# facebookresearch/SlowFast

Measured on NVIDIA H100. Metric: clips/sec (fwd+bwd) SlowFast-8x8-R50, higher is better.
Workload: dtype bf16x3-split operands, f32 accumulate/storage

## Files before the change

include/slowfast_b200.h:

```cpp
#ifndef SLOWFAST_B200_H_
#define SLOWFAST_B200_H_

#include <stdint.h>

#ifdef __cplusplus
extern "C" {
#endif

const char* sfb_last_error(void);
int sfb_abi_version(void);
const char* sfb_build_arch(void);

typedef struct sfb_conv_desc {
  const void* a_hi;
  const void* a_lo;
  int32_t n, d, h, w, c;
  int64_t c_pitch;
  const void* b_hi;
  const void* b_lo;
  int32_t cout;
  int32_t kt, kh, kw;
  int32_t dil_t, dil_h, dil_w;
  int32_t str_t, str_h, str_w;
  int32_t low_t, low_h, low_w;
  int32_t out_t, out_h, out_w;
  float* out;
  int64_t os_n, os_t, os_h, os_w;
  int32_t accumulate;
  float* stats;
  int32_t nsplit;
} sfb_conv_desc;

int64_t sfb_conv_m_tiles(const sfb_conv_desc* d);
int32_t sfb_conv_ksplit(const sfb_conv_desc* d);
int sfb_conv_igemm(const sfb_conv_desc* d, void* stream);

typedef struct sfb_wgrad_desc {
  const void* x_hi;
  const void* x_lo;
  int32_t n, d, h, w, c;
  int64_t c_pitch;
  const void* dy_hi;
  const void* dy_lo;
  int32_t cout;
  int64_t dy_pitch;
  int32_t kt, kh, kw;
  int32_t dil_t, dil_h, dil_w;
  int32_t str_t, str_h, str_w;
  int32_t low_t, low_h, low_w;
  int32_t out_t, out_h, out_w;
  float* dw;
  int32_t nsplit;
} sfb_wgrad_desc;

int sfb_conv_wgrad(const sfb_wgrad_desc* d, void* stream);

typedef struct sfb_wgrad_plan {
  int32_t direct;
  int32_t transposed;
  int32_t tile_rows;
  int32_t bn;
  int32_t ck;
  int32_t tiles;
  int32_t k_blocks;
  int32_t slices;
  int32_t ctas;
} sfb_wgrad_plan;
int sfb_conv_wgrad_plan(const sfb_wgrad_desc* d, int32_t num_sms, sfb_wgrad_plan* out);

int sfb_set_wgrad_direct(int32_t enabled);

int sfb_zero_f32_2d(float* ptr, int64_t rows, int64_t c, int64_t pitch, void* stream);

int sfb_add_f32_2d(float* dst, const float* src, int64_t rows, int32_t c, int64_t dst_pitch, int64_t src_pitch,
                   void* stream);

int sfb_split_planes(const float* x, int64_t rows, int32_t c, int64_t x_pitch, void* hi, void* lo,
                     int64_t o_pitch, void* stream);
int sfb_input_pack(const float* x, int32_t n, int32_t c, int32_t t, int32_t h, int32_t w, int32_t c_pad, void* hi,
                   void* lo, void* stream);
int sfb_filter_pack(const float* w, int32_t cout, int32_t cin, int32_t taps_total, const int32_t* tapmap,
                    int32_t ntaps, int32_t transpose, int32_t cols_pad, void* hi, void* lo, void* stream);
int sfb_filter_unpack_grad(const float* dwm, float* dw, int32_t cout, int32_t cin, int32_t taps, int32_t cin_pad,
                           int32_t accumulate, void* stream);

int sfb_bn_finalize(const float* partials, int32_t m_tiles, int32_t c, int64_t count, const float* gamma,
                    const float* beta, float* running_mean, float* running_var, float momentum, float eps,
                    int32_t training, float* scale, float* shift, float* save_mean, float* save_invstd,
                    int32_t affine_c, void* stream);

int32_t sfb_bn_split_stats_tiles(int64_t rows, int64_t rows_per_clip, int32_t splits, int32_t c);
int sfb_bn_split_stats(const float* y, int64_t y_pitch, int64_t rows, int32_t c, int32_t splits, int64_t rows_per_clip,
                       float* partials, void* stream);

typedef struct sfb_bn_apply_desc {
  const float* y; int64_t y_pitch; const float* scale; const float* shift;
  const float* y2; int64_t y2_pitch; const float* scale2; const float* shift2;
  const void* res_hi; const void* res_lo; int64_t res_pitch;
  void* out_hi; void* out_lo; int64_t out_pitch;
  int64_t rows; int32_t c; int32_t relu;
  int32_t splits; int64_t rows_per_clip;
} sfb_bn_apply_desc;
int sfb_bn_apply(const sfb_bn_apply_desc* d, void* stream);

typedef struct sfb_bn_bwd_desc {
  const float* dout; int64_t dout_pitch;
  const void* mask_hi; int64_t mask_pitch;
  const float* y; int64_t y_pitch;
  const float* mean; const float* invstd; const float* gamma;
  float* dgamma; float* dbeta; int32_t accumulate_param_grads;
  int32_t training;
  void* dy_hi; void* dy_lo; int64_t dy_pitch;
  float* dres; int64_t dres_pitch; int32_t dres_accumulate;
  float* partials;
  float* coef;
  int64_t rows; int32_t c;
  int32_t c_valid;
  const float* mask_scale; const float* mask_shift;
  int32_t splits; int64_t rows_per_clip;
} sfb_bn_bwd_desc;
int32_t sfb_bn_bwd_blocks(int64_t rows, int32_t c, int32_t splits, int64_t rows_per_clip);
int sfb_bn_bwd(const sfb_bn_bwd_desc* d, void* stream);

typedef struct sfb_pool_desc {
  const float* y; const float* scale; const float* shift;
  int32_t n, t, h, w, c, oh, ow, kh, kw, sh, sw, ph, pw;
  void* out_hi; void* out_lo; int64_t out_pitch;
  uint8_t* argmax;
  const float* dout; int64_t dout_pitch;
  float* dz;
  int32_t splits;
} sfb_pool_desc;
int sfb_bn_relu_maxpool_fwd(const sfb_pool_desc* d, void* stream);
int sfb_bn_relu_maxpool_bwd(const sfb_pool_desc* d, void* stream);



typedef struct sfb_pool3d_desc {
  const void* in_hi; const void* in_lo; int64_t in_pitch;
  void* out_hi; void* out_lo; int64_t out_pitch;
  uint8_t* argmax;
  int32_t n, t, h, w, c, ot, oh, ow;
  int32_t kt, kh, kw, st, sh, sw, pt, ph, pw;
  const float* dout; int64_t dout_pitch;
  float* din; int64_t din_pitch; int32_t din_accumulate;
} sfb_pool3d_desc;
int sfb_maxpool3d_fwd(const sfb_pool3d_desc* d, void* stream);
int sfb_maxpool3d_bwd(const sfb_pool3d_desc* d, void* stream);

int sfb_stem_input_fold(const float* x, int32_t n, int32_t cin, int32_t t, int32_t h, int32_t w, void* hi, void* lo,
                        void* stream);
int sfb_stem_filter_fold(const float* w, float* dw, int32_t cout, int32_t cin, int32_t kt, int32_t kh, int32_t kw,
                         int32_t pad_w, int32_t kwf, void* hi, void* lo, const float* gmat, int32_t reverse,
                         void* stream);
typedef struct sfb_stem_desc {
  const void* x_hi; const void* x_lo;
  int32_t n, t, h, wf;
  const void* f_hi; const void* f_lo;
  const void* dy_hi; const void* dy_lo;
  int32_t cout, kt, kh, kwf;
  int32_t str_t, str_h, pad_t, pad_h, pad_wf;
  int32_t out_t, out_h, out_w;
  float* out;
  float* stats;
  float* dwm;
  int32_t nsplit;
} sfb_stem_desc;
int64_t sfb_stem_m_tiles(const sfb_stem_desc* d);
int sfb_stem_fprop(const sfb_stem_desc* d, void* stream);
int sfb_stem_wgrad(const sfb_stem_desc* d, void* stream);
int sfb_stem8_supported(const sfb_stem_desc* d);
int64_t sfb_stem8_m_tiles(const sfb_stem_desc* d);
int sfb_stem8_input_fold(const float* x, int32_t n, int32_t cin, int32_t t, int32_t h, int32_t w, void* hi, void* lo,
                         void* stream);
int sfb_stem8_filter_fold(const float* w, int32_t cin, int32_t kt, void* hi, void* lo, void* stream);
int sfb_stem8_fprop(const sfb_stem_desc* d, void* stream);
int sfb_stem8_wgrad(const sfb_stem_desc* d, void* stream);

typedef struct sfb_bgemm_desc {
  const void* a_hi; const void* a_lo; int64_t lda, batch_stride_a; int32_t a_mn_major;
  const void* b_hi; const void* b_lo; int64_t ldb, batch_stride_b; int32_t b_mn_major;
  int32_t m, n, k, batch;
  float* out; int64_t ldd, batch_stride_d;
  float alpha;
  int32_t accumulate;
  int32_t nsplit;
} sfb_bgemm_desc;
int sfb_gemm_batched(const sfb_bgemm_desc* d, void* stream);

int sfb_layernorm_fwd(const float* x, int64_t x_pitch, int64_t rows, int32_t c, const float* gamma, const float* beta,
                      float eps, void* o_hi, void* o_lo, float* o_f32, int64_t o_pitch, float* mean, float* rstd,
                      void* stream);
int32_t sfb_rowslab_blocks(int64_t rows);
int sfb_layernorm_bwd(const float* dy, int64_t dy_pitch, const float* x, int64_t x_pitch, int64_t rows, int32_t c,
                      const float* gamma, const float* mean, const float* rstd, float* dx, int64_t dx_pitch,
                      int32_t dx_accumulate, float* dgamma, float* dbeta, int32_t param_accumulate, float* partials,
                      void* stream);
int sfb_colsum(const float* src, int64_t pitch, int64_t rows, int32_t c, float* out, int32_t accumulate, float* partials,
               void* stream);
int sfb_tokens_assemble(const float* y, const float* bias, const float* cls, const float* pos_spatial,
                        const float* pos_temporal, const float* pos_class, int32_t b, int32_t l, int32_t hw, int32_t c,
                        float* x, void* stream);
// ... 211 lines not shown
```

slowfast_b200/csrc/conv_direct.cu:

```cuda
#include <cstdint>
#include <cuda_bf16.h>

#include "../../include/slowfast_b200.h"
#include "tmap.h"

namespace sfb {

struct DirectParams {
  const __nv_bfloat16* a_hi; const __nv_bfloat16* a_lo; int64_t c_pitch;
  const __nv_bfloat16* b_hi; const __nv_bfloat16* b_lo;
  int nb, id, ih, iw, c, cout;
  int kd, kh, kw, dd, dh, dw, sd, sh, sw, ld, lh, lw, oz, op, oq;
  int M, m_tiles, ktot, coutp;
  float* out; long long os_n, os_z, os_p, os_q; int accumulate; int ncols_store;
  float* stats;
};

__device__ __forceinline__ void dc_load8(const __nv_bfloat16* hi, const __nv_bfloat16* lo, int64_t off, float (&x)[8]) {
  const uint4 h = *reinterpret_cast<const uint4*>(hi + off);
  const uint32_t hw[4] = {h.x, h.y, h.z, h.w};
#pragma unroll
  for (int i = 0; i < 4; ++i) {
    x[2 * i] = __uint_as_float(hw[i] << 16);
    x[2 * i + 1] = __uint_as_float(hw[i] & 0xffff0000u);
// ... 49 lines not shown
          const int iw = w0 + tw * p.dw;
          if (id < 0 || id >= p.id || ih < 0 || ih >= p.ih || iw < 0 || iw >= p.iw) continue;
          const int64_t base = (((int64_t(on_) * p.id + id) * p.ih + ih) * p.iw + iw) * p.c_pitch;
          const float* wt = wsm + size_t(tap) * p.c * COUT_T;
          for (int c0 = 0; c0 < p.c; c0 += 8) {
            float x[8];
            dc_load8(p.a_hi, p.a_lo, base + c0, x);
#pragma unroll
            for (int ci = 0; ci < 8; ++ci) {
              const float xv = x[ci];
              const float4* w4 = reinterpret_cast<const float4*>(wt + size_t(c0 + ci) * COUT_T);
#pragma unroll
              for (int j = 0; j < COUT_T / 4; ++j) {
                const float4 w = w4[j];
                acc[4 * j + 0] = fmaf(xv, w.x, acc[4 * j + 0]);
                acc[4 * j + 1] = fmaf(xv, w.y, acc[4 * j + 1]);
                acc[4 * j + 2] = fmaf(xv, w.z, acc[4 * j + 2]);
                acc[4 * j + 3] = fmaf(xv, w.w, acc[4 * j + 3]);
              }
            }
          }
        }
      }
    }
  }
  float* tile = red + 8 * COUT_T;
  long long* roff_s = reinterpret_cast<long long*>(tile + 128 * (COUT_T + 1));
#pragma unroll
  for (int j = 0; j < COUT_T; ++j) tile[threadIdx.x * (COUT_T + 1) + j] = acc[j];
  roff_s[threadIdx.x] = rvalid ? roff : -1;
  __syncthreads();
  {
    const int ncols = p.ncols_store;
    for (int e = threadIdx.x; e < 128 * ncols; e += 128) {
      int px, col;
      if (ncols == COUT_T) {
        px = e / COUT_T;
        col = e - px * COUT_T;
      } else {
        px = e / ncols;
        col = e - px * ncols;
      }
      const long long off = roff_s[px];
      if (off < 0) continue;
      float v = tile[px * (COUT_T + 1) + col];
      float* dst = p.out + off + col;
      if (p.accumulate == 2) {
        atomicAdd(dst, v);
      } else {
        if (p.accumulate) v += *dst;
        *dst = v;
      }
    }
  }
  if (p.stats == nullptr) return;
  const int lane = threadIdx.x & 31, warp = threadIdx.x >> 5;
#pragma unroll
  for (int j = 0; j < COUT_T; ++j) {
    float s = rvalid ? acc[j] : 0.f;
    float s2 = s * s;
#pragma unroll
    for (int o = 16; o > 0; o >>= 1) {
      s += __shfl_xor_sync(0xffffffffu, s, o);
      s2 += __shfl_xor_sync(0xffffffffu, s2, o);
    }
    if (lane == 0) {
      red[(warp * 2 + 0) * COUT_T + j] = s;
      red[(warp * 2 + 1) * COUT_T + j] = s2;
    }
  }
  __syncthreads();
  for (int j = threadIdx.x; j < p.cout; j += blockDim.x) {
    float s = 0.f, s2 = 0.f;
#pragma unroll
    for (int w = 0; w < 4; ++w) {
      s += red[(w * 2 + 0) * COUT_T + j];
      s2 += red[(w * 2 + 1) * COUT_T + j];
    }
    p.stats[size_t(j) * p.m_tiles + mt] = s;
    p.stats[(size_t(p.cout) + j) * p.m_tiles + mt] = s2;
  }
}

int conv_direct_try(const sfb_conv_desc* d, cudaStream_t stream, int* rc_out) {
  const int taps = d->kt * d->kh * d->kw;
  const int64_t macs = int64_t(taps) * d->c * d->cout;
  int coutp = 8;
  while (coutp < d->cout) coutp <<= 1;
  const size_t smem = (size_t(taps) * d->c * coutp + size_t(8) * coutp + size_t(128) * (coutp + 1)) * sizeof(float) +
                      128 * sizeof(long long) + 8;
  if (d->c > 8 || d->cout > 64 || macs > 1024 || smem > 96 * 1024) return 0;
  DirectParams p;
  p.a_hi = (const __nv_bfloat16*)d->a_hi; p.a_lo = (const __nv_bfloat16*)d->a_lo; p.c_pitch = d->c_pitch;
  p.b_hi = (const __nv_bfloat16*)d->b_hi; p.b_lo = (const __nv_bfloat16*)d->b_lo;
  p.nb = d->n; p.id = d->d; p.ih = d->h; p.iw = d->w; p.c = d->c; p.cout = d->cout;
  p.kd = d->kt; p.kh = d->kh; p.kw = d->kw; p.dd = d->dil_t; p.dh = d->dil_h; p.dw = d->dil_w;
  p.sd = d->str_t; p.sh = d->str_h; p.sw = d->str_w; p.ld = d->low_t; p.lh = d->low_h; p.lw = d->low_w;
  p.oz = d->out_t; p.op = d->out_h; p.oq = d->out_w;
  p.M = int(int64_t(d->n) * d->out_t * d->out_h * d->out_w);
  p.m_tiles = (p.M + 127) / 128;
  p.ktot = taps * d->c;
  p.coutp = coutp;
  p.out = d->out; p.os_n = d->os_n; p.os_z = d->os_t; p.os_p = d->os_h; p.os_q = d->os_w;
  p.accumulate = d->accumulate;
  p.ncols_store = (d->cout + 3) & ~3;
  p.stats = d->stats;
  static bool attr = false;
  if (!attr) {
    cudaFuncSetAttribute(conv_direct_kernel<8>, cudaFuncAttributeMaxDynamicSharedMemorySize, 100 * 1024);
    cudaFuncSetAttribute(conv_direct_kernel<16>, cudaFuncAttributeMaxDynamicSharedMemorySize, 100 * 1024);
    cudaFuncSetAttribute(conv_direct_kernel<32>, cudaFuncAttributeMaxDynamicSharedMemorySize, 100 * 1024);
    cudaFuncSetAttribute(conv_direct_kernel<64>, cudaFuncAttributeMaxDynamicSharedMemorySize, 100 * 1024);
    attr = true;
  }
  switch (coutp) {
    case 8: conv_direct_kernel<8><<<p.m_tiles, 128, smem, stream>>>(p); break;
    case 16: conv_direct_kernel<16><<<p.m_tiles, 128, smem, stream>>>(p); break;
    case 32: conv_direct_kernel<32><<<p.m_tiles, 128, smem, stream>>>(p); break;
    default: conv_direct_kernel<64><<<p.m_tiles, 128, smem, stream>>>(p); break;
  }
  const cudaError_t e = cudaGetLastError();
  if (e != cudaSuccess) {
    set_error("sfb_conv_igemm (direct SIMT body) launch failed: %s", cudaGetErrorString(e));
    *rc_out = -20;
  } else {
    *rc_out = 0;
  }
  return 1;
}

}
```

slowfast_b200/csrc/conv_igemm.cu:

```cuda
#include <algorithm>
#include <cstdint>
#include <cstdio>

#include "../../include/slowfast_b200.h"
#include "ptx.cuh"
#include "tmap.h"

namespace sfb {

constexpr int BLOCK_M = 128;
constexpr int MAX_STAGES = 8;
constexpr int EPI_WARPS = 8;
constexpr int EPI_STAGE_FLOATS = 64;
constexpr int MMA_WARPS = 8;
constexpr int PRODUCER_WARP = MMA_WARPS;
constexpr int EPI_WARP0 = MMA_WARPS + 1;
constexpr int CONV_THREADS = 32 * (MMA_WARPS + 1 + EPI_WARPS);
constexpr int BN_MAX = 128;
constexpr int BLOCK_K = 64;
constexpr int KSTEPS = BLOCK_K / 16;

struct ConvParams {
  CUtensorMap tmA[2];
  CUtensorMap tmB[2];
  int M, oq, op, oz, nb;
  int sw, sh, sd;
  int lw, lh, ld;
  int kw, kh, kd;
  int dw, dh, dd;
  int CK, cpt, n_chunks, cps, k_blocks;
  int Ntot, BN, n_tiles, m_tiles;
  int ksplit;
  int stages;
  int a_tiled;
  uint32_t stage_bytes, chunk_bytes, b_bytes, a_total_bytes, a_plane_bytes;
  uint32_t a_layout, a_sbo, a_lbo;
  uint32_t a_kstep[KSTEPS];
  uint32_t acc_pitch;
  uint32_t off_acc, off_staging, off_red, off_bars;
  float* out;
  long long os_n, os_z, os_p, os_q;
  int accumulate;
  int epi_coalesced;
  float* stats;
};

__device__ __forceinline__ int k_block_begin(const ConvParams& p, int kpart) {
  return kpart * p.k_blocks / p.ksplit;
}

int conv_direct_try(const sfb_conv_desc* d, cudaStream_t stream, int* rc_out);

template <int NSPLIT, int BN>
__global__ void __launch_bounds__(CONV_THREADS, 1) conv_igemm_kernel(const __grid_constant__ ConvParams p) {
  static_assert(BN % 16 == 0 && BN <= BN_MAX, "tile width: a multiple of 16 up to BN_MAX");
  extern __shared__ uint8_t smem_raw[];
  uint8_t* smem = reinterpret_cast<uint8_t*>((reinterpret_cast<uintptr_t>(smem_raw) + 1023) & ~uintptr_t(1023));

  const int warp = threadIdx.x >> 5;
  const int lane = threadIdx.x & 31;

  uint64_t* full = reinterpret_cast<uint64_t*>(smem + p.off_bars);
  uint64_t* empty = full + MAX_STAGES;
  uint64_t* tfull = empty + MAX_STAGES;
  uint64_t* tempty = tfull + 1;
  float* acc_tile = reinterpret_cast<float*>(smem + p.off_acc);

  if (threadIdx.x == 0) {
    for (int s = 0; s < p.stages; ++s) {
      mbar_init(&full[s], 1);
      mbar_init(&empty[s], 32 * MMA_WARPS);
    }
    mbar_init(tfull, 32 * MMA_WARPS);
    mbar_init(tempty, EPI_WARPS);
    fence_mbar_init();
    fence_proxy_async_smem();
  }
  __syncthreads();

  const int total_units = p.m_tiles * p.n_tiles * p.ksplit;

  if (warp == PRODUCER_WARP) {
    if (lane == 0) {
      tma_prefetch_desc(&p.tmA[0]);
      tma_prefetch_desc(&p.tmB[0]);
      if (NSPLIT == 3) {
        tma_prefetch_desc(&p.tmA[1]);
        tma_prefetch_desc(&p.tmB[1]);
      }
    }
    int stage = 0;
    uint32_t phase = 0;
    for (int unit = blockIdx.x; unit < total_units; unit += gridDim.x) {
      const int tile = unit / p.ksplit, kpart = unit - tile * p.ksplit;
      const int mt = tile / p.n_tiles, nt = tile - mt * p.n_tiles;
      const int kb0 = k_block_begin(p, kpart), kb1 = k_block_begin(p, kpart + 1);
      int t = mt * BLOCK_M;
      const int q0 = t % p.oq;
      t /= p.oq;
      const int p0 = t % p.op;
      t /= p.op;
      const int z0 = t % p.oz;
      const int n0 = t / p.oz;
      const int cw = p.lw + q0 * p.sw, ch = p.lh + p0 * p.sh, cd = p.ld + z0 * p.sd;
      for (int kb = kb0; kb < kb1; ++kb) {
        mbar_wait(&empty[stage], phase ^ 1);
        if (elect_one()) {
          const int chunk0 = kb * p.cps;
          const uint32_t bytes = (uint32_t(p.cps) * p.chunk_bytes + p.b_bytes) * (NSPLIT == 3 ? 2u : 1u);
          mbar_expect_tx(&full[stage], bytes);
          uint8_t* st = smem + size_t(stage) * p.stage_bytes;
          for (int j = 0; j < p.cps; ++j) {
            const int idx = chunk0 + j;
            int nn = p.nb, c0 = 0;
            uint16_t ow = 0, oh = 0, od = 0;
            if (idx < p.n_chunks) {
              const int tap = idx / p.cpt;
              c0 = (idx - tap * p.cpt) * p.CK;
              const int tw = tap % p.kw;
              const int t2 = tap / p.kw;
              const int th = t2 % p.kh;
              const int td = t2 / p.kh;
              ow = uint16_t(tw * p.dw);
              oh = uint16_t(th * p.dh);
              od = uint16_t(td * p.dd);
              nn = n0;
            }
            if (p.a_tiled) {
              const int row0 = idx < p.n_chunks ? mt * BLOCK_M : p.m_tiles * BLOCK_M;
              tma_load_2d(st + j * p.chunk_bytes, &p.tmA[0], &full[stage], c0, row0);
              if (NSPLIT == 3) tma_load_2d(st + p.a_plane_bytes + j * p.chunk_bytes, &p.tmA[1], &full[stage], c0, row0);
              continue;
            }
            tma_load_im2col_5d(st + j * p.chunk_bytes, &p.tmA[0], &full[stage], c0, cw, ch, cd, nn, ow, oh, od);
            if (NSPLIT == 3)
              tma_load_im2col_5d(st + p.a_plane_bytes + j * p.chunk_bytes, &p.tmA[1], &full[stage], c0, cw, ch, cd,
                                 nn, ow, oh, od);
          }
          tma_load_2d(st + p.a_total_bytes, &p.tmB[0], &full[stage], kb * 64, nt * BN);
          if (NSPLIT == 3)
            tma_load_2d(st + p.a_total_bytes + p.b_bytes, &p.tmB[1], &full[stage], kb * 64, nt * BN);
        }
        __syncwarp();
        if (++stage == p.stages) {
          stage = 0;
          phase ^= 1;
        }
      }
    }
  } else if (warp < MMA_WARPS) {
    const int g = warp >> 2;
    const uint32_t a_row_off = uint32_t(g) * 8u * p.a_sbo;
    float d[BN / 2];
    int stage = 0;
    uint32_t phase = 0;
    int it = 0;
    for (int unit = blockIdx.x; unit < total_units; unit += gridDim.x, ++it) {
      const int kpart = unit % p.ksplit;
      const int kb0 = k_block_begin(p, kpart), kb1 = k_block_begin(p, kpart + 1);
#pragma unroll
      for (int i = 0; i < BN / 2; ++i) d[i] = 0.f;
      int held = -1;
      for (int kb = kb0; kb < kb1; ++kb) {
        mbar_wait(&full[stage], phase);
        wgmma_fence();
        const uint32_t a_base = smem_u32(smem + size_t(stage) * p.stage_bytes) + a_row_off;
        const uint32_t b_base = smem_u32(smem + size_t(stage) * p.stage_bytes) + p.a_total_bytes;
        const uint64_t a_hi0 = make_smem_desc(a_base, p.a_lbo, p.a_sbo, p.a_layout);
        const uint64_t b_hi0 = make_smem_desc(b_base, 16, 1024, 2);
#pragma unroll
        for (int ks = 0; ks < KSTEPS; ++ks) {
          const uint64_t a_hi = a_hi0 + p.a_kstep[ks];
          const uint64_t b_hi = b_hi0 + uint64_t(ks * 2);
          if (NSPLIT == 3) {
            const uint64_t a_lo = a_hi + (p.a_plane_bytes >> 4);
            const uint64_t b_lo = b_hi + (p.b_bytes >> 4);
            wgmma_m64n<BN>(d, a_lo, b_hi);
            wgmma_m64n<BN>(d, a_hi, b_lo);
          }
          wgmma_m64n<BN>(d, a_hi, b_hi);
        }
        wgmma_commit();
        wgmma_wait<1>();
        if (held >= 0) mbar_arrive(&empty[held]);
        held = stage;
        if (++stage == p.stages) {
          stage = 0;
          phase ^= 1;
        }
      }
      wgmma_wait<0>();
      mbar_arrive(&empty[held]);
      mbar_wait(tempty, (it & 1) ^ 1);
      acc_store<BN>(d, BN, acc_tile + size_t(g) * 64 * p.acc_pitch, int(p.acc_pitch));
      mbar_arrive(tfull);
    }
  } else {
    const int ew = warp - EPI_WARP0;
    const int q = ew & 3;
    const int half = ew >> 2;
    long long* roff_s = reinterpret_cast<long long*>(reinterpret_cast<float*>(smem + p.off_staging) + ew * EPI_STAGE_FLOATS);
    float* red = reinterpret_cast<float*>(smem + p.off_red);
    const int sub = lane >> 2, cq = lane & 3;
    constexpr int nchunks = BN >> 4;
    const float* qtile = acc_tile + size_t(q) * 32 * p.acc_pitch;
    int it = 0;
    for (int unit = blockIdx.x; unit < total_units; unit += gridDim.x, ++it) {
      const int tile = unit / p.ksplit;
      const int acc = it & 1;
      const int mt = tile / p.n_tiles, nt = tile - mt * p.n_tiles;
      const int ncol0 = nt * BN;
      const int row = mt * BLOCK_M + q * 32 + lane;
      const bool rvalid = row < p.M;
      long long roff = 0;
      if (rvalid) {
        int t = row;
        const int oq_ = t % p.oq;
        t /= p.oq;
        const int op_ = t % p.op;
        t /= p.op;
        const int oz_ = t % p.oz;
        const int on_ = t / p.oz;
        roff = on_ * p.os_n + oz_ * p.os_z + op_ * p.os_p + oq_ * p.os_q;
      }
      const uint32_t rmask = __ballot_sync(0xffffffffu, rvalid);
      float* red_w = red + ((size_t(acc) * 4 + q) * BN) * 2;
      roff_s[lane] = roff;
      __syncwarp();
      long long ro[4];
#pragma unroll
      for (int k = 0; k < 4; ++k) ro[k] = roff_s[k * 8 + sub];

      mbar_wait(tfull, it & 1);
      for (int ch = half; ch < nchunks; ch += 2) {
        const int c0 = ch * 16;
        const int limit = min(BN, p.Ntot - ncol0) - c0;
        const bool cvalid = cq * 4 < limit;
        float s4[4] = {0.f, 0.f, 0.f, 0.f}, q4[4] = {0.f, 0.f, 0.f, 0.f};
#pragma unroll
        for (int k = 0; k < 4; ++k) {
          const int r = k * 8 + sub;
          const float4 y = *reinterpret_cast<const float4*>(qtile + size_t(r) * p.acc_pitch + c0 + cq * 4);
          s4[0] += y.x; s4[1] += y.y; s4[2] += y.z; s4[3] += y.w;
          q4[0] = fmaf(y.x, y.x, q4[0]); q4[1] = fmaf(y.y, y.y, q4[1]);
          q4[2] = fmaf(y.z, y.z, q4[2]); q4[3] = fmaf(y.w, y.w, q4[3]);
          if (((rmask >> r) & 1u) && cvalid) {
            float4* dst = reinterpret_cast<float4*>(p.out + ro[k] + ncol0 + c0 + cq * 4);
            if (p.accumulate == 2) {
              asm volatile("red.global.add.v4.f32 [%0], {%1, %2, %3, %4};" ::"l"(dst), "f"(y.x), "f"(y.y), "f"(y.z), "f"(y.w)
                           : "memory");
            } else if (p.accumulate) {
              const float4 o = *dst;
              *dst = make_float4(y.x + o.x, y.y + o.y, y.z + o.z, y.w + o.w);
            } else {
              *dst = y;
            }
          }
        }
        if (p.stats != nullptr) {
#pragma unroll
          for (int i = 0; i < 4; ++i) {
#pragma unroll
            for (int o = 4; o <= 16; o <<= 1) {
              s4[i] += __shfl_xor_sync(0xffffffffu, s4[i], o);
              q4[i] += __shfl_xor_sync(0xffffffffu, q4[i], o);
            }
          }
          if (sub == 0) {
#pragma unroll
            for (int i = 0; i < 4; ++i) {
              const int cl = c0 + cq * 4 + i;
              red_w[cl * 2 + 0] = s4[i];
              red_w[cl * 2 + 1] = q4[i];
            }
          }
        }
      }
      __syncwarp();
      if (lane == 0) mbar_arrive(tempty);
      if (p.stats != nullptr) {
        named_bar_sync(1, 32 * EPI_WARPS);
        const float* rb = red + size_t(acc) * 4 * BN * 2;
        for (int cl = ew * 32 + lane; cl < BN; cl += 32 * EPI_WARPS) {
          const int col = ncol0 + cl;
          if (col < p.Ntot) {
            float s = 0.f, s2 = 0.f;
#pragma unroll
            for (int w = 0; w < 4; ++w) {
              s += rb[(size_t(w) * BN + cl) * 2 + 0];
              s2 += rb[(size_t(w) * BN + cl) * 2 + 1];
            }
            p.stats[size_t(col) * p.m_tiles + mt] = s;
            p.stats[(size_t(p.Ntot) + col) * p.m_tiles + mt] = s2;
          }
        }
      }
    }
  }

}

static int g_num_sms = 0;
static int g_smem_optin = 0;

static int device_props() {
  if (g_num_sms) return 0;
  int dev = 0;
  if (cudaGetDevice(&dev) != cudaSuccess) {
    set_error("cudaGetDevice failed: no CUDA device");
    return -1;
  }
  cudaDeviceGetAttribute(&g_num_sms, cudaDevAttrMultiProcessorCount, dev);
  cudaDeviceGetAttribute(&g_smem_optin, cudaDevAttrMaxSharedMemoryPerBlockOptin, dev);
  return 0;
}

static int pick_ck(int c) {
  if (c % 64 == 0) return 64;
  if (c % 32 == 0) return 32;
  if (c % 16 == 0) return 16;
  return 8;
}

struct ConvGrid {
  int64_t M;
  int CK, cps, n_chunks, k_blocks, BN, m_tiles, n_tiles;
};
static ConvGrid conv_grid(const sfb_conv_desc* d) {
  ConvGrid g;
  g.M = int64_t(d->n) * d->out_t * d->out_h * d->out_w;
  g.CK = pick_ck(d->c);
  g.cps = BLOCK_K / g.CK;
  g.n_chunks = d->kt * d->kh * d->kw * (d->c / g.CK);
  g.k_blocks = (g.n_chunks + g.cps - 1) / g.cps;
  g.BN = std::min((d->cout + 15) / 16 * 16, BN_MAX);
  g.m_tiles = int((g.M + BLOCK_M - 1) / BLOCK_M);
  g.n_tiles = (d->cout + g.BN - 1) / g.BN;
  return g;
}

static bool rows_regular(const sfb_conv_desc* d) {
  return d->os_h == int64_t(d->out_w) * d->os_w && d->os_t == int64_t(d->out_h) * d->os_h &&
         d->os_n == int64_t(d->out_t) * d->os_t;
}

static int conv_ksplit(const sfb_conv_desc* d, const ConvGrid& g, bool with_stats) {
  const int tiles = g.m_tiles * g.n_tiles;
  const int P = g_num_sms;
  if (P <= 0 || d->c <= 8 || 2 * tiles < P) return 1;
  if ((d->accumulate == 0 || with_stats) && !rows_regular(d)) return 1;
  if (with_stats && (d->accumulate != 0 || d->cout % 8 != 0 || d->os_w % 4 != 0)) return 1;
  auto cost = [&](int s) { return double((int64_t(tiles) * s + P - 1) / P) / s * (1.0 + 0.02 * (s - 1)); };
  int best = 1;
  for (int s = 2; s <= 8 && 4 * s <= g.k_blocks; ++s)
    if (cost(s) < cost(best)) best = s;
  return cost(best) < 0.9 * cost(1) ? best : 1;
}

}

using namespace sfb;

extern "C" int64_t sfb_conv_m_tiles(const sfb_conv_desc* d) {
  const ConvGrid g = conv_grid(d);
  if (device_props() == 0 && conv_ksplit(d, g, true) > 1)
    return sfb_bn_split_stats_tiles(g.M, g.M, 1, d->cout);
  return g.m_tiles;
}

extern "C" int32_t sfb_conv_ksplit(const sfb_conv_desc* d) {
  if (device_props()) return 1;
  return conv_ksplit(d, conv_grid(d), d->stats != nullptr);
}

extern "C" int sfb_conv_igemm(const sfb_conv_desc* d, void* stream_) {
  cudaStream_t stream = reinterpret_cast<cudaStream_t>(stream_);
  if (device_props()) return -1;
  if (d->nsplit != 1 && d->nsplit != 3) {
    set_error("sfb_conv_igemm: nsplit must be 1 or 3 (got %d)", d->nsplit);
    return -10;
  }
  if (d->c % 8 != 0 || d->c_pitch % 8 != 0 || d->c <= 0) {
    set_error("sfb_conv_igemm: channel count %d / pitch %lld must be positive multiples of 8", d->c,
              (long long)d->c_pitch);
    return -10;
  }
  if (!d->a_hi || !d->b_hi || !d->out || (d->nsplit == 3 && (!d->a_lo || !d->b_lo))) {
    set_error("sfb_conv_igemm: null operand pointer");
    return -10;
  }
  const int64_t M64 = int64_t(d->n) * d->out_t * d->out_h * d->out_w;
  if (M64 <= 0 || M64 > 0x7fffffffLL || d->cout <= 0) {
    set_error("sfb_conv_igemm: bad output extent M=%lld cout=%d", (long long)M64, d->cout);
    return -10;
  }

  {
    int rc_direct = 0;
    if (conv_direct_try(d, stream, &rc_direct)) return rc_direct;
  }
  ConvParams p;
  memset(&p, 0, sizeof(p));
  p.M = int(M64);
  p.oq = d->out_w;
  p.op = d->out_h;
  p.oz = d->out_t;
  p.nb = d->n;
  p.sw = d->str_w;
  p.sh = d->str_h;
  p.sd = d->str_t;
  p.lw = d->low_w;
  p.lh = d->low_h;
  p.ld = d->low_t;
  p.kw = d->kw;
  p.kh = d->kh;
  p.kd = d->kt;
  p.dw = d->dil_w;
  p.dh = d->dil_h;
  p.dd = d->dil_t;
  const ConvGrid g = conv_grid(d);
  const int taps = d->kt * d->kh * d->kw;
  p.CK = g.CK;
  p.cpt = d->c / p.CK;
  p.n_chunks = g.n_chunks;
  p.cps = g.cps;
  p.k_blocks = g.k_blocks;
  p.Ntot = d->cout;
  p.BN = g.BN;
  p.n_tiles = g.n_tiles;
  p.m_tiles = g.m_tiles;
  p.ksplit = conv_ksplit(d, g, d->stats != nullptr);
  p.chunk_bytes = BLOCK_M * p.CK * 2;
  p.b_bytes = p.BN * 128;
  p.a_plane_bytes = (uint32_t(p.cps) * p.chunk_bytes + 1023u) / 1024u * 1024u;
  p.a_total_bytes = p.a_plane_bytes * (d->nsplit == 3 ? 2 : 1);
  p.stage_bytes = p.a_total_bytes + p.b_bytes * (d->nsplit == 3 ? 2 : 1);
  p.stage_bytes = (p.stage_bytes + 1023) / 1024 * 1024;
  switch (p.CK) {
    case 64: p.a_layout = 2; p.a_sbo = 1024; p.a_lbo = 16; break;
    case 32: p.a_layout = 4; p.a_sbo = 512; p.a_lbo = 16; break;
    case 16: p.a_layout = 6; p.a_sbo = 256; p.a_lbo = 16; break;
    default: p.a_layout = 0; p.a_sbo = 128; p.a_lbo = p.chunk_bytes; break;
  }
  for (int ks = 0; ks < KSTEPS; ++ks) {
    const int k0 = ks * 16;
    const uint32_t off = p.CK >= 16 ? uint32_t(k0 / p.CK) * p.chunk_bytes + uint32_t(k0 % p.CK) * 2u
                                    : uint32_t(ks * 2) * p.chunk_bytes;
    p.a_kstep[ks] = off >> 4;
  }
  p.acc_pitch = uint32_t(p.BN) + 4;
  const uint32_t acc_bytes = BLOCK_M * p.acc_pitch * 4;
  const uint32_t tail = acc_bytes + EPI_WARPS * EPI_STAGE_FLOATS * 4 + 2 * 4 * p.BN * 2 * 4 + 256;
  const uint32_t budget = uint32_t(g_smem_optin) - 1024 - tail;
  p.stages = std::min<int>(MAX_STAGES, budget / p.stage_bytes);
  p.stages = std::min(p.stages, std::max(2, p.k_blocks * 4));
  const int ctas_per_sm = 1;
  if (p.stages < 2) {
    set_error("sfb_conv_igemm: not enough shared memory for 2 pipeline stages (stage=%u B)", p.stage_bytes);
    return -11;
  }
  p.off_acc = p.stages * p.stage_bytes;
  p.off_staging = p.off_acc + acc_bytes;
  p.off_red = p.off_staging + EPI_WARPS * EPI_STAGE_FLOATS * 4;
  p.off_bars = p.off_red + 2 * 4 * p.BN * 2 * 4;
  const uint32_t smem_bytes = p.off_bars + 256 + 1024;
  p.out = d->out;
  p.os_n = d->os_n;
  p.os_z = d->os_t;
  p.os_p = d->os_h;
  p.os_q = d->os_w;
  p.accumulate = p.ksplit > 1 ? 2 : d->accumulate;
  p.epi_coalesced = 1;
  p.stats = p.ksplit > 1 ? nullptr : d->stats;

  const int lower[3] = {d->low_w, d->low_h, d->low_t};
  const int strd[3] = {d->str_w, d->str_h, d->str_t};
  const int upper[3] = {d->low_w + (d->out_w - 1) * d->str_w + 1 - d->w, d->low_h + (d->out_h - 1) * d->str_h + 1 - d->h,
                        d->low_t + (d->out_t - 1) * d->str_t + 1 - d->d};
  const SwizzleBytes aswz = p.CK == 64 ? SWZ_128 : p.CK == 32 ? SWZ_64 : p.CK == 16 ? SWZ_32 : SWZ_NONE;
  p.a_tiled = (taps == 1 && d->str_w == 1 && d->str_h == 1 && d->str_t == 1 && d->low_w == 0 && d->low_h == 0 &&
               d->low_t == 0 && d->out_w == d->w && d->out_h == d->h && d->out_t == d->d)
                  ? 1 : 0;
  int rc;
  if (p.a_tiled)
    rc = make_tmap_2d_bf16(&p.tmA[0], d->a_hi, uint64_t(p.M), uint64_t(d->c), uint64_t(d->c_pitch), BLOCK_M, p.CK, aswz);
  else
    rc = make_tmap_im2col_bf16(&p.tmA[0], d->a_hi, d->n, d->d, d->h, d->w, d->c, d->c_pitch, lower, upper, strd, p.CK,
                               BLOCK_M, aswz);
  if (rc) return rc;
  const uint64_t ktot = uint64_t(taps) * d->c;
  rc = make_tmap_2d_bf16(&p.tmB[0], d->b_hi, d->cout, ktot, ktot, p.BN, 64, SWZ_128);
  if (rc) return rc;
  if (d->nsplit == 3) {
    if (p.a_tiled)
      rc = make_tmap_2d_bf16(&p.tmA[1], d->a_lo, uint64_t(p.M), uint64_t(d->c), uint64_t(d->c_pitch), BLOCK_M, p.CK, aswz);
    else
      rc = make_tmap_im2col_bf16(&p.tmA[1], d->a_lo, d->n, d->d, d->h, d->w, d->c, d->c_pitch, lower, upper, strd,
                                 p.CK, BLOCK_M, aswz);
    if (rc) return rc;
    rc = make_tmap_2d_bf16(&p.tmB[1], d->b_lo, d->cout, ktot, ktot, p.BN, 64, SWZ_128);
    if (rc) return rc;
  }

  if (p.ksplit > 1 && d->accumulate == 0) {
    const size_t width = size_t((d->cout + 3) & ~3) * sizeof(float);
    if (cudaMemset2DAsync(d->out, size_t(d->os_w) * sizeof(float), 0, width, size_t(p.M), stream) != cudaSuccess) {
      set_error("sfb_conv_igemm: zero fill of the split-K output failed: %s", cudaGetErrorString(cudaGetLastError()));
      return -20;
    }
  }
  const int units = p.m_tiles * p.n_tiles * p.ksplit;
  const int grid = std::min(units, g_num_sms * ctas_per_sm);
  {
    typedef void (*KernelFn)(const ConvParams);
#define SFB_CONV_FNS(S) {conv_igemm_kernel<S, 16>, conv_igemm_kernel<S, 32>, conv_igemm_kernel<S, 48>, \
                         conv_igemm_kernel<S, 64>, conv_igemm_kernel<S, 80>, conv_igemm_kernel<S, 96>, \
                         conv_igemm_kernel<S, 112>, conv_igemm_kernel<S, 128>}
    static const KernelFn fns[2][BN_MAX / 16] = {SFB_CONV_FNS(1), SFB_CONV_FNS(3)};
#undef SFB_CONV_FNS
    static bool attr[2][BN_MAX / 16] = {};
    const int a = d->nsplit == 3 ? 1 : 0, b = p.BN / 16 - 1;
    if (!attr[a][b]) {
      cudaFuncSetAttribute(fns[a][b], cudaFuncAttributeMaxDynamicSharedMemorySize, g_smem_optin);
      attr[a][b] = true;
    }
    fns[a][b]<<<grid, CONV_THREADS, smem_bytes, stream>>>(p);
  }
  cudaError_t e = cudaGetLastError();
  if (e != cudaSuccess) {
    set_error("sfb_conv_igemm launch failed: %s (grid=%d smem=%u stages=%d BN=%d CK=%d ksplit=%d)",
              cudaGetErrorString(e), grid, smem_bytes, p.stages, p.BN, p.CK, p.ksplit);
    return -20;
  }
  if (p.ksplit > 1 && d->stats != nullptr)
    return sfb_bn_split_stats(d->out, d->os_w, p.M, d->cout, 1, p.M, d->stats, stream);
  return 0;
}
```

slowfast_b200/csrc/elementwise.cu:

```cuda
#include <cstdint>
#include <cstring>
#include <cuda_bf16.h>

#include "../../include/slowfast_b200.h"
#include "tmap.h"

namespace sfb {

static int ew_sms() {
  static int sms = 0;
  if (!sms) {
    int dev = 0;
    if (cudaGetDevice(&dev) != cudaSuccess) return 148;
    cudaDeviceGetAttribute(&sms, cudaDevAttrMultiProcessorCount, dev);
  }
  return sms;
}
static int ew_grid(int64_t items, int block) {
  int64_t want = (items + block - 1) / block;
  int64_t cap = int64_t(ew_sms()) * 8;
  return int(want < 1 ? 1 : (want > cap ? cap : want));
}
static int rowlane_grid(int64_t rows, int cg, int block) {
  const int lanes_c = cg < block ? cg : block;
// ... 375 lines not shown
#pragma unroll
          for (int j = 0; j < 8; ++j) d[j] = fmaf(yv[j], msc[j], msh[j]) > 0.f ? d[j] : 0.f;
        }
#pragma unroll
        for (int j = 0; j < 8; ++j) {
          s1[j] += d[j];
          s2[j] = fmaf(d[j], (yv[j] - mu[j]) * is[j], s2[j]);
        }
      }
    }
#pragma unroll
    for (int j = 0; j < 8; ++j) {
      sm[threadIdx.x * 16 + j] = s1[j];
      sm[threadIdx.x * 16 + 8 + j] = s2[j];
    }
    __syncthreads();
    if (lr == 0 && g < cg) {
      for (int k = 1; k < lanes_r; ++k) {
#pragma unroll
        for (int j = 0; j < 8; ++j) {
          s1[j] += sm[(k * lanes_c + lc) * 16 + j];
          s2[j] += sm[(k * lanes_c + lc) * 16 + 8 + j];
        }
      }
      float* out = p.partials + size_t(blockIdx.x) * 2 * p.c;
      store8(out + g * 8, s1);
      store8(out + p.c + g * 8, s2);
    }
    __syncthreads();
  }
}

__global__ void __launch_bounds__(64) bn_bwd_finalize_kernel(const float* __restrict__ partials, int nblocks, int c,
                                                             double count, const float* __restrict__ gamma,
                                                             const float* __restrict__ invstd,
                                                             float* __restrict__ dgamma, float* __restrict__ dbeta,
                                                             int accumulate, int training,
                                                             float* __restrict__ coef , int c_valid,
                                                             int splits, int blocks_per_clip) {
  __shared__ double sm1[64], sm2[64];
  const int ch = blockIdx.x;
  const int sc = splits * c;
  if (ch >= c_valid) {
    if (threadIdx.x == 0)
      for (int s = 0; s < splits; ++s) coef[s * c + ch] = coef[sc + s * c + ch] = coef[2 * sc + s * c + ch] = 0.f;
    return;
  }
  const int nb_split = nblocks / splits;
  double t1 = 0.0, t2 = 0.0;
  for (int s = 0; s < splits; ++s) {
    double s1 = 0.0, s2 = 0.0;
    for (int i = threadIdx.x; i < nb_split; i += 64) {
      const int b = splits > 1 ? ((i / blocks_per_clip) * splits + s) * blocks_per_clip + i % blocks_per_clip : i;
      s1 += double(partials[size_t(b) * 2 * c + ch]);
      s2 += double(partials[size_t(b) * 2 * c + c + ch]);
    }
    sm1[threadIdx.x] = s1;
    sm2[threadIdx.x] = s2;
    __syncthreads();
    for (int o = 32; o > 0; o >>= 1) {
      if (threadIdx.x < o) {
        sm1[threadIdx.x] += sm1[threadIdx.x + o];
        sm2[threadIdx.x] += sm2[threadIdx.x + o];
      }
      __syncthreads();
    }
    if (threadIdx.x == 0) {
      s1 = sm1[0];
      s2 = sm2[0];
      t1 += s1;
      t2 += s2;
      const double a = double(gamma ? gamma[ch] : 1.f) * double(invstd[s * c + ch]);
      coef[s * c + ch] = float(a);
      coef[sc + s * c + ch] = training ? float(a * s1 / count) : 0.f;
      coef[2 * sc + s * c + ch] = training ? float(a * s2 / count) : 0.f;
    }
    __syncthreads();
  }
  if (threadIdx.x != 0) return;
  if (dgamma) dgamma[ch] = accumulate ? dgamma[ch] + float(t2) : float(t2);
  if (dbeta) dbeta[ch] = accumulate ? dbeta[ch] + float(t1) : float(t1);
}

struct BnBwdApplyParams {
  const float* dout; int64_t dout_pitch;
  const __nv_bfloat16* mask; int64_t mask_pitch;
  const float* y; int64_t y_pitch;
  const float* mean; const float* invstd; const float* coef;
  __nv_bfloat16* dy_hi; __nv_bfloat16* dy_lo; int64_t dy_pitch;
  float* dres; int64_t dres_pitch; int dres_accumulate;
  int64_t rows; int c;
  const float* mask_scale; const float* mask_shift;
  int splits; int64_t rows_per_clip;
};
struct BnBwdCoef {
  float mu[8], ca[8], cb[8], k1[8], msc[8], msh[8];
  __device__ __forceinline__ void load(const BnBwdApplyParams& p, int s, int c) {
    const int64_t o = int64_t(s) * p.c + c, sc = int64_t(p.splits > 1 ? p.splits : 1) * p.c;
    float is[8], cc[8];
    load8(p.mean + o, mu);
    load8(p.invstd + o, is);
    load8(p.coef + o, ca);
    load8(p.coef + sc + o, cb);
    load8(p.coef + 2 * sc + o, cc);
#pragma unroll
    for (int j = 0; j < 8; ++j) k1[j] = is[j] * cc[j];
    if (p.mask_scale) {
      load8(p.mask_scale + o, msc);
      load8(p.mask_shift + o, msh);
    }
  }
};
__global__ void __launch_bounds__(256) bn_bwd_apply_kernel(const BnBwdApplyParams p) {
  const int cg = p.c / 8;
  const RowLanes L(cg);
  if (L.lr >= L.lanes_r) return;
  for (int g = L.lc; g < cg; g += L.lanes_c) {
    const int c = g * 8;
    BnBwdCoef k;
    k.load(p, 0, c);
    float (&mu)[8] = k.mu, (&ca)[8] = k.ca, (&cb)[8] = k.cb, (&k1)[8] = k.k1, (&msc)[8] = k.msc, (&msh)[8] = k.msh;
    int cur = 0;
    for (int64_t r = int64_t(blockIdx.x) * L.lanes_r + L.lr; r < p.rows; r += int64_t(gridDim.x) * L.lanes_r) {
      if (p.splits > 1) {
        const int s = split_of_row(r, p.rows_per_clip, p.splits);
        if (s != cur) {
          cur = s;
          k.load(p, s, c);
        }
      }
      float d[8], yv[8];
      load8(p.dout + r * p.dout_pitch + c, d);
      load8(p.y + r * p.y_pitch + c, yv);
      if (p.mask) {
        float m[8];
        load_planes8(p.mask + r * p.mask_pitch + c, nullptr, m);
#pragma unroll
        for (int j = 0; j < 8; ++j) d[j] = m[j] > 0.f ? d[j] : 0.f;
      } else if (p.mask_scale) {
#pragma unroll
        for (int j = 0; j < 8; ++j) d[j] = fmaf(yv[j], msc[j], msh[j]) > 0.f ? d[j] : 0.f;
      }
      if (p.dres) {
        float* dr = p.dres + r * p.dres_pitch + c;
        if (p.dres_accumulate) {
          float o[8];
          load8(dr, o);
#pragma unroll
          for (int j = 0; j < 8; ++j) o[j] += d[j];
          store8(dr, o);
        } else {
          store8(dr, d);
        }
      }
      float gq[8];
#pragma unroll
      for (int j = 0; j < 8; ++j) gq[j] = ca[j] * d[j] - cb[j] - (yv[j] - mu[j]) * k1[j];
      store_split8(p.dy_hi + r * p.dy_pitch + c, p.dy_lo ? p.dy_lo + r * p.dy_pitch + c : nullptr, gq);
    }
  }
}

struct PoolParams {
  const float* y; const float* scale; const float* shift;
  int n, t, h, w, c; int oh, ow; int kh, kw, sh, sw, ph, pw;
  __nv_bfloat16* o_hi; __nv_bfloat16* o_lo; int64_t o_pitch;
// ... 182 lines not shown
  }
  return 1;
}

extern "C" int32_t sfb_bn_split_stats_tiles(int64_t rows, int64_t rows_per_clip, int32_t splits, int32_t c) {
  if (rows_per_clip <= 0 || splits <= 0 || c < 8) return 0;
  const int64_t chunk = split_stats_chunk(c);
  const int64_t chunks = (rows_per_clip + chunk - 1) / chunk;
  return int32_t(rows / rows_per_clip / splits * chunks);
}

extern "C" int sfb_bn_split_stats(const float* y, int64_t y_pitch, int64_t rows, int32_t c, int32_t splits,
                                  int64_t rows_per_clip, float* partials, void* stream) {
  if (c % 8 || y_pitch % 4 || splits < 1 || rows_per_clip <= 0 || rows % rows_per_clip ||
      (rows / rows_per_clip) % splits) {
    set_error("sfb_bn_split_stats: c=%d (a multiple of 8), %lld rows in clips of %lld rows, %d splits", c,
              (long long)rows, (long long)rows_per_clip, splits);
    return -10;
  }
  SplitStatsParams p;
  p.y = y; p.y_pitch = y_pitch; p.rows_per_clip = rows_per_clip; p.chunk_rows = split_stats_chunk(c);
  p.c = c; p.splits = splits;
  p.chunks = int((rows_per_clip + p.chunk_rows - 1) / p.chunk_rows);
  p.blocks_per_split = sfb_bn_split_stats_tiles(rows, rows_per_clip, splits, c);
  p.partials = partials;
  const int64_t blocks = rows / rows_per_clip * p.chunks;
  if (blocks == 0) return 0;
  bn_split_stats_kernel<<<unsigned(blocks), 256, 256 * 16 * sizeof(float), (cudaStream_t)stream>>>(p);
  SFB_LAUNCH_CHECK("sfb_bn_split_stats");
  return 0;
}

extern "C" int sfb_bn_apply(const sfb_bn_apply_desc* d, void* stream) {
  if (d->c % 8) {
    set_error("sfb_bn_apply: c=%d must be a multiple of 8", d->c);
    return -10;
  }
  if (!split_geometry_ok("sfb_bn_apply", d->rows, d->splits, d->rows_per_clip)) return -10;
  BnApplyParams p;
  p.y = d->y; p.y_pitch = d->y_pitch; p.scale = d->scale; p.shift = d->shift;
  p.y2 = d->y2; p.y2_pitch = d->y2_pitch; p.scale2 = d->scale2; p.shift2 = d->shift2;
  p.r_hi = (const bf16*)d->res_hi; p.r_lo = (const bf16*)d->res_lo; p.r_pitch = d->res_pitch;
  p.o_hi = (bf16*)d->out_hi; p.o_lo = (bf16*)d->out_lo; p.o_pitch = d->out_pitch;
  p.rows = d->rows; p.c = d->c; p.relu = d->relu;
  p.splits = d->splits > 1 ? d->splits : 1; p.rows_per_clip = d->rows_per_clip;
  const int64_t items = d->rows * (d->c / 8);
  if (items == 0) return 0;
  bn_apply_kernel<<<rowlane_grid(d->rows, d->c / 8, 256), 256, 0, (cudaStream_t)stream>>>(p);
  SFB_LAUNCH_CHECK("sfb_bn_apply");
  return 0;
}

static int64_t bn_bwd_slabs(int64_t rows) {
  int64_t b = (rows + 15) / 16;
  const int64_t cap = int64_t(ew_sms()) * 4;
  if (b > cap) b = cap;
  if (b < 1) b = 1;
  return b;
}

static int32_t bn_bwd_blocks_per_clip(int64_t rows, int64_t rows_per_clip) {
  const int64_t clips = rows / rows_per_clip;
  int64_t per = (bn_bwd_slabs(rows) + clips - 1) / clips;
  const int64_t most = (rows_per_clip + 15) / 16;
  if (per > most) per = most;
  return int32_t(per < 1 ? 1 : per);
}

extern "C" int32_t sfb_bn_bwd_blocks(int64_t rows, int32_t c, int32_t splits, int64_t rows_per_clip) {
  (void)c;
  if (splits > 1 && rows_per_clip > 0)
    return int32_t(rows / rows_per_clip * bn_bwd_blocks_per_clip(rows, rows_per_clip));
  return int32_t(bn_bwd_slabs(rows));
}

extern "C" int sfb_bn_bwd(const sfb_bn_bwd_desc* d, void* stream_) {
  cudaStream_t stream = (cudaStream_t)stream_;
  if (d->c % 8) {
    set_error("sfb_bn_bwd: c=%d must be a multiple of 8", d->c);
    return -10;
  }
  if (!split_geometry_ok("sfb_bn_bwd", d->rows, d->splits, d->rows_per_clip)) return -10;
  const int splits = d->splits > 1 ? d->splits : 1;
  const int nblocks = sfb_bn_bwd_blocks(d->rows, d->c, splits, d->rows_per_clip);
  const int bpc = splits > 1 ? bn_bwd_blocks_per_clip(d->rows, d->rows_per_clip) : 1;
  BnBwdReduceParams r;
  r.dout = d->dout; r.dout_pitch = d->dout_pitch;
  r.mask = (const bf16*)d->mask_hi; r.mask_pitch = d->mask_pitch;
  r.mask_scale = d->mask_scale; r.mask_shift = d->mask_shift;
  r.y = d->y; r.y_pitch = d->y_pitch; r.mean = d->mean; r.invstd = d->invstd;
  r.rows = d->rows; r.c = d->c; r.partials = d->partials;
  r.splits = splits; r.rows_per_clip = d->rows_per_clip; r.blocks_per_clip = bpc;
  bn_bwd_reduce_kernel<<<nblocks, 256, 256 * 16 * sizeof(float), stream>>>(r);
  SFB_LAUNCH_CHECK("sfb_bn_bwd(reduce)");
  bn_bwd_finalize_kernel<<<d->c, 64, 0, stream>>>(d->partials, nblocks, d->c, double(d->rows / splits), d->gamma,
                                                                 d->invstd, d->dgamma, d->dbeta, d->accumulate_param_grads,
                                                                 d->training, d->coef,
                                                                 d->c_valid > 0 ? d->c_valid : d->c, splits, bpc);
  SFB_LAUNCH_CHECK("sfb_bn_bwd(finalize)");
  BnBwdApplyParams a;
  a.dout = d->dout; a.dout_pitch = d->dout_pitch;
  a.mask = (const bf16*)d->mask_hi; a.mask_pitch = d->mask_pitch;
  a.mask_scale = d->mask_scale; a.mask_shift = d->mask_shift;
  a.y = d->y; a.y_pitch = d->y_pitch; a.mean = d->mean; a.invstd = d->invstd; a.coef = d->coef;
  a.dy_hi = (bf16*)d->dy_hi; a.dy_lo = (bf16*)d->dy_lo; a.dy_pitch = d->dy_pitch;
  a.dres = d->dres; a.dres_pitch = d->dres_pitch; a.dres_accumulate = d->dres_accumulate;
  a.rows = d->rows; a.c = d->c;
  a.splits = splits; a.rows_per_clip = d->rows_per_clip;
  const int64_t items = d->rows * (d->c / 8);
  bn_bwd_apply_kernel<<<rowlane_grid(d->rows, d->c / 8, 256), 256, 0, stream>>>(a);
  SFB_LAUNCH_CHECK("sfb_bn_bwd(apply)");
  return 0;
}

extern "C" int sfb_bn_relu_maxpool_fwd(const sfb_pool_desc* d, void* stream) {
  if (d->c % 8 || d->kh * d->kw > 254) {
    set_error("sfb_bn_relu_maxpool_fwd: c=%d must be a multiple of 8 and the window < 255 taps", d->c);
    return -10;
  }
  PoolParams p;
  memset(&p, 0, sizeof(p));
  p.y = d->y; p.scale = d->scale; p.shift = d->shift;
  p.n = d->n; p.t = d->t; p.h = d->h; p.w = d->w; p.c = d->c; p.oh = d->oh; p.ow = d->ow;
  p.kh = d->kh; p.kw = d->kw; p.sh = d->sh; p.sw = d->sw; p.ph = d->ph; p.pw = d->pw;
  p.o_hi = (bf16*)d->out_hi; p.o_lo = (bf16*)d->out_lo; p.o_pitch = d->out_pitch; p.argmax = d->argmax;
  p.splits = d->splits > 1 ? d->splits : 1;
  if (d->n % p.splits) {
    set_error("sfb_bn_relu_maxpool_fwd: batch %d is not a multiple of %d splits", d->n, p.splits);
    return -10;
  }
  const int64_t items = int64_t(d->n) * d->t * d->oh * d->ow * (d->c / 8);
  bn_relu_maxpool_fwd_kernel<<<ew_grid(items, 256), 256, 0, (cudaStream_t)stream>>>(p);
  SFB_LAUNCH_CHECK("sfb_bn_relu_maxpool_fwd");
  return 0;
}

extern "C" int sfb_bn_relu_maxpool_bwd(const sfb_pool_desc* d, void* stream) {
  if (d->c % 8) {
    set_error("sfb_bn_relu_maxpool_bwd: c=%d must be a multiple of 8", d->c);
    return -10;
  }
  PoolParams p;
  memset(&p, 0, sizeof(p));
  p.n = d->n; p.t = d->t; p.h = d->h; p.w = d->w; p.c = d->c; p.oh = d->oh; p.ow = d->ow;
  p.kh = d->kh; p.kw = d->kw; p.sh = d->sh; p.sw = d->sw; p.ph = d->ph; p.pw = d->pw;
  p.argmax = d->argmax; p.dout = d->dout; p.dout_pitch = d->dout_pitch; p.dz = d->dz;
  const int64_t items = int64_t(d->n) * d->t * d->h * d->w * (d->c / 8);
  bn_relu_maxpool_bwd_kernel<<<ew_grid(items, 256), 256, 0, (cudaStream_t)stream>>>(p);
  SFB_LAUNCH_CHECK("sfb_bn_relu_maxpool_bwd");
  return 0;
}

namespace sfb {
struct Pool3dParams {
  const __nv_bfloat16* i_hi; const __nv_bfloat16* i_lo; int64_t i_pitch;
  __nv_bfloat16* o_hi; __nv_bfloat16* o_lo; int64_t o_pitch;
  uint8_t* argmax;
  int n, t, h, w, c, ot, oh, ow;
  int kt, kh, kw, st, sh, sw, pt, ph, pw;
  const float* dout; int64_t dout_pitch; float* din; int64_t din_pitch; int din_accumulate;
};
__global__ void maxpool3d_fwd_kernel(const Pool3dParams p) {
  const int cg = p.c / 8;
  const int64_t items = int64_t(p.n) * p.ot * p.oh * p.ow * cg;
  for (int64_t i = blockIdx.x * int64_t(blockDim.x) + threadIdx.x; i < items; i += int64_t(gridDim.x) * blockDim.x) {
    const int g = int(i % cg);
    int64_t pos = i / cg;
    const int ox = int(pos % p.ow);
    int64_t r = pos / p.ow;
    const int oy = int(r % p.oh);
    r /= p.oh;
    const int oz = int(r % p.ot);
    const int64_t b = r / p.ot;
    const int c = g * 8;
    float best[8];
    uint8_t arg[8];
#pragma unroll
    for (int j = 0; j < 8; ++j) { best[j] = -INFINITY; arg[j] = 0; }
    for (int kz = 0; kz < p.kt; ++kz) {
      const int iz = oz * p.st - p.pt + kz;
      if (iz < 0 || iz >= p.t) continue;
      for (int ky = 0; ky < p.kh; ++ky) {
// ... 138 lines not shown
```

slowfast_b200/engine.py:

```python
from __future__ import annotations

from typing import Dict, List, Optional, Sequence, Tuple

import torch
import torch.nn as nn

from . import ops
from .conv_plan import dgrad_out_view, dgrad_plan
from .ops import F32, F32View, Planes
from .subbn import is_sub_bn


class Storage:

    def __init__(self, n, t, h, w, pitch, nsplit, device, planes: bool = True):
        self.shape = (n, t, h, w, pitch)
        self.hi = torch.empty(self.shape if planes else (0, 0, 0, 0, pitch), dtype=torch.bfloat16, device=device)
        self.lo = torch.empty(self.shape, dtype=torch.bfloat16, device=device) if (nsplit == 3 and planes) else None
        self.grad: Optional[torch.Tensor] = None
        self.grad_written = False

    def ensure_grad(self) -> torch.Tensor:
        if self.grad is None:
            self.grad = torch.empty(self.shape, dtype=F32, device=self.hi.device)
# ... 66 lines not shown
                victim = min(live, key=lambda k: self._arenas[k].last_use)
                old = self._arenas.pop(victim)
                for cb in old.on_evict:
                    cb()
        self._arena_clock = getattr(self, "_arena_clock", 0) + 1
        a.last_use = self._arena_clock
        self.arena = a
        self._bufs, self._storages, self._scratch = a.bufs, a.storages, a.scratch
        return a

    def buf(self, key: Tuple, shape: Sequence[int], dtype=F32, zero: bool = False) -> torch.Tensor:
        t = self._bufs.get(key)
        if t is None or tuple(t.shape) != tuple(shape) or t.dtype != dtype:
            t = (torch.zeros if zero else torch.empty)(tuple(shape), dtype=dtype, device=self.device)
            self._bufs[key] = t
        return t

    def storage(self, key: Tuple, n, t, h, w, pitch, planes: bool = True) -> Storage:
        s = self._storages.get(key)
        if s is None or s.shape != (n, t, h, w, pitch):
            s = Storage(n, t, h, w, pitch, self.nsplit, self.device, planes)
            self._storages[key] = s
        return s

    def scratch(self, tag: str, nelem: int, dtype) -> torch.Tensor:
        t = self._scratch.get(tag)
        if t is None or t.numel() < nelem or t.dtype != dtype:
            t = torch.empty(int(nelem), dtype=dtype, device=self.device)
            self._scratch[tag] = t
        return t[:nelem]

    def scratch_planes(self, tag: str, n, t, h, w, c) -> Planes:
        nelem = n * t * h * w * c
        hi = self.scratch(tag + ".hi", nelem, torch.bfloat16).view(n, t, h, w, c)
        lo = self.scratch(tag + ".lo", nelem, torch.bfloat16).view(n, t, h, w, c) if self.nsplit == 3 else None
        return Planes(hi, lo, n, t, h, w, c, 0)

    def begin_backward(self, params: Sequence[nn.Parameter]) -> None:
        offsets, total = flat_offsets(params)
        self.flat_grad = torch.zeros(total, dtype=F32, device=self.device) if total != sum(p.numel() for p in params) \
            else torch.empty(total, dtype=F32, device=self.device)
        self.grad_slots = {}
        for p, off in zip(params, offsets):
            self.grad_slots[id(p)] = self.flat_grad[off:off + p.numel()].view(p.shape)
        for s in self._storages.values():
            s.grad_written = False

    def grad_of(self, p: nn.Parameter) -> torch.Tensor:
        return self.grad_slots[id(p)]


FLAT_ALIGN = 64


def flat_offsets(params: Sequence[nn.Parameter], align: int = FLAT_ALIGN) -> Tuple[List[int], int]:
    offsets, off = [], 0
    for p in params:
        offsets.append(off)
        off += (p.numel() + align - 1) // align * align
    return offsets, off


def allreduce_flat_gradients(flat: torch.Tensor, params: Sequence[nn.Parameter], group=None,
                             repoint: bool = True) -> None:
    import torch.distributed as dist
    world = dist.get_world_size(group)
    if dist.get_backend(group) == "nccl":
        dist.all_reduce(flat, op=dist.ReduceOp.AVG, group=group)
    else:
        dist.all_reduce(flat, op=dist.ReduceOp.SUM, group=group)
        flat.div_(world)
    if not repoint:
        return
    offsets, total = flat_offsets(params)
    assert total == flat.numel(), "flat bucket does not match the parameter list"
    for p, off in zip(params, offsets):
        n = p.numel()
        if p.grad is None or p.grad.data_ptr() != flat.data_ptr() + flat.element_size() * off:
            p.grad = flat[off:off + n].view_as(p)


def _t3(v) -> Tuple[int, int, int]:
    return tuple(int(x) for x in v)


class ConvBN:

    def __init__(self, name: str, conv: nn.Conv3d, bn: Optional[nn.Module], ctx: Ctx):
        assert conv.groups == 1 and _t3(conv.dilation) == (1, 1, 1), \
            f"{name}: only dense, undilated Conv3d is on this path"
        self.name, self.conv, self.bn, self.ctx = name, conv, bn, ctx
        self.bias = conv.bias
        self.sub = bn is not None and is_sub_bn(bn)
        assert bn is None or self._stats_bn(True).momentum is not None, \
            f"{name}: BatchNorm momentum=None (cumulative moving average) is not on the engine path"
        assert not self.sub or (bn.affine and conv.out_channels % 8 == 0), \
            f"{name}: sub-batch BN needs an affine container and a multiple of 8 channels"
        self.splits, self.rows_per_clip = 1, 0
        self.k, self.stride, self.pad = _t3(conv.kernel_size), _t3(conv.stride), _t3(conv.padding)
        self.cin, self.cout = conv.in_channels, conv.out_channels
        self.cin_pad = ops.pad8(self.cin)
        self.cout_pad = ops.pad8(self.cout)
        self.taps = self.k[0] * self.k[1] * self.k[2]
        self.x: Optional[Planes] = None
        self.geom = None
        self.y: Optional[torch.Tensor] = None

    def out_dims(self, t, h, w):
        return tuple(ops.conv_out_size(i, k, s, p) for i, k, s, p in zip((t, h, w), self.k, self.stride, self.pad))

    def _stats_bn(self, training: bool) -> nn.Module:
        if not self.sub:
            return self.bn
        return self.bn.split_bn if training else self.bn.bn

    @property
    def split_kw(self) -> dict:
        return {"splits": self.splits, "rows_per_clip": self.rows_per_clip}

    def _bn_forward(self, y: torch.Tensor, stats: Optional[torch.Tensor], m_tiles: int, cp: int, zero: bool) -> None:
        ctx, bn, c, s = self.ctx, self.bn, self.cout, self.splits
        rows = y.numel() // y.shape[-1]
        if s > 1:
            m_tiles = ops.bn_split_stats_tiles(rows, self.rows_per_clip, s, c)
            stats = ctx.buf((self.name, "stats.split"), (2, s * c, m_tiles))
            ops.bn_split_stats(ops.f32view(y), s, self.rows_per_clip, stats)
        self.scale = ctx.buf((self.name, "scale"), (s * cp,), zero=zero)
        self.shift = ctx.buf((self.name, "shift"), (s * cp,), zero=zero)
        self.mean = ctx.buf((self.name, "mean"), (s * cp,), zero=zero)
        self.invstd = ctx.buf((self.name, "invstd"), (s * cp,), zero=zero)
        sbn = self._stats_bn(ctx.training)
        momentum = sbn.momentum if sbn.momentum is not None else 0.1
        ops.bn_finalize(stats, m_tiles, s * c, rows // s, bn.weight, bn.bias, sbn.running_mean, sbn.running_var,
                        momentum, sbn.eps, ctx.training, self.scale, self.shift, self.mean, self.invstd, affine_c=c)
        if self.bias is not None:
            ops.bn_conv_bias(self.bias, c, momentum, ctx.training, sbn.running_mean, self.scale, self.shift, self.mean,
                             splits=s)

    def fprop(self, x: Planes) -> torch.Tensor:
        ctx = self.ctx
        assert x.c == self.cin_pad, (self.name, x.c, self.cin_pad)
        geom = ops.fprop_geom(x, self.k, self.stride, self.pad)
        ot, oh, ow = geom.out
        f = ctx.buf((self.name, "f.hi"), (self.cout, self.taps * self.cin_pad), torch.bfloat16)
        flo = ctx.buf((self.name, "f.lo"), f.shape, torch.bfloat16) if ctx.nsplit == 3 else None
        fm = ops.FilterMat(f, flo, self.cout, self.taps, self.cin_pad)
        ops.filter_pack(self.conv.weight, fm)
        c, cp = self.cout, self.cout_pad
        y = ctx.buf((self.name, "y"), (x.n, ot, oh, ow, cp))
        strides = (ot * oh * ow * cp, oh * ow * cp, ow * cp, cp)
        m_tiles = ops.conv_stats_tiles(x, fm, geom, y, strides, nsplit=ctx.nsplit)
        self.splits = self.bn.num_splits if (self.sub and ctx.training) else 1
        self.rows_per_clip = ot * oh * ow
        stats = ctx.buf((self.name, "stats"), (2, c, m_tiles)) \
            if (ctx.training and self.bn is not None and self.splits == 1) else None
        ops.conv_igemm(x, fm, geom, y, strides, stats=stats, nsplit=ctx.nsplit)
        self.x, self.geom, self.y = x, geom, y
        if self.bn is None:
            return y
        self._bn_forward(y, stats, m_tiles, cp, zero=True)
        return y

    def bwd(self, dout: F32View, mask: Optional[Planes], x_act: Optional[Act], dres: Optional[F32View] = None,
            dres_accumulate: bool = False, mask_from_y: bool = False) -> None:
        ctx = self.ctx
        n, ot, oh, ow, c = self.y.shape
        dy = ctx.scratch_planes("dy", n, ot, oh, ow, c)
        partials, coef = self._bwd_scratch(n * ot * oh * ow, c)
        bn = self.bn
        ops.bn_bwd(dout, mask, ops.f32view(self.y), self.mean, self.invstd, bn.weight, ctx.grad_of(bn.weight),
                   ctx.grad_of(bn.bias), dy, partials, coef, training=ctx.training, dres=dres,
                   dres_accumulate=dres_accumulate, c_valid=self.cout,
                   mask_affine=(self.scale, self.shift) if mask_from_y else None, **self.split_kw)
        if self.bias is not None:
            rows = n * ot * oh * ow
            dyf = ctx.scratch("bias.dy", rows * c, F32).view(rows, c)
            ops.planes_to_f32(dy, ops.f32view(dyf))
            part = ctx.scratch("colsum.part", ops.colsum_blocks(rows) * self.cout, F32)
            ops.colsum(dyf, rows, self.cout, ctx.grad_of(self.bias), part, pitch=c)
        self.wgrad(dy)
        if x_act is not None:
            self.dgrad(dy, x_act)

    def _bwd_scratch(self, rows, c):
        nb = ops.bn_bwd_blocks(rows, c, self.splits, self.rows_per_clip)
        return (self.ctx.scratch("bnb.partials", nb * 2 * c, F32).view(nb, 2, c),
                self.ctx.scratch("bnb.coef", 3 * self.splits * c, F32).view(3, self.splits * c))

    def wgrad(self, dy: Planes) -> None:
        ctx = self.ctx
        gw = ctx.grad_of(self.conv.weight)
        if self.taps == 1 and self.cin_pad == self.cin and self.cout_pad == self.cout:
            ops.zero_f32(ops.f32view(gw.view(self.cout, self.cin)))
            ops.conv_wgrad(self.x, dy, self.geom, gw, nsplit=ctx.nsplit)
        else:
            dwm = ctx.scratch("dwm", self.cout_pad * self.taps * self.cin_pad, F32).view(self.cout_pad, -1)
            ops.zero_f32(ops.f32view(dwm))
            ops.conv_wgrad(self.x, dy, self.geom, dwm, nsplit=ctx.nsplit)
            ops.filter_unpack_grad(dwm, gw, self.cin_pad, accumulate=False)

    def dgrad(self, dy: Planes, x_act: Act) -> None:
        ctx = self.ctx
        _, t, h, w, pitch = x_act.s.shape
        plan = dgrad_plan((t, h, w), self.k, self.stride, self.pad)
        acc = x_act.s.grad_written
        g = x_act.s.ensure_grad()
        if plan.needs_zero_fill and not acc:
            ops.zero_f32(x_act.grad_view())
        for sub in plan.subs:
            ntap = len(sub.tapmap)
            cp = ops.pad8(self.cout)
            f = ctx.scratch("dgf.hi", self.cin * ntap * cp, torch.bfloat16).view(self.cin, ntap * cp)
            flo = ctx.scratch("dgf.lo", self.cin * ntap * cp, torch.bfloat16).view(self.cin, ntap * cp) \
                if ctx.nsplit == 3 else None
            fm = ops.FilterMat(f, flo, self.cin, ntap, cp)
            ops.filter_pack(self.conv.weight, fm, tapmap=sub.tapmap, transpose=True)
            off, strides = dgrad_out_view((t, h, w), self.stride, sub, pitch, x_act.c0)
            ops.conv_igemm(dy, fm, ops.ConvGeom(sub.k, (1, 1, 1), sub.low, sub.out), g, strides, out_offset=off,
                           accumulate=2 if acc else 0, nsplit=ctx.nsplit)
        x_act.s.grad_written = True


class StemConvBN(ConvBN):

    def __init__(self, name, conv, bn, ctx):
        super().__init__(name, conv, bn, ctx)
        self.g = ops.StemGeom(self.cin, self.cout, self.k, self.stride, self.pad)
        self.t8 = False

    @staticmethod
    def supported(conv: nn.Conv3d, w: int) -> bool:
        return (conv.out_channels <= 64 and conv.out_channels % 8 == 0 and
                ops.stem_supported(conv.in_channels, _t3(conv.kernel_size), _t3(conv.stride), _t3(conv.padding), w))

    def pack_input(self, x: torch.Tensor, key) -> "Act":
        n, c, t, h, w = x.shape
        x_f32 = x.contiguous().float()
        self.t8 = bool(self.cout == 8 and
                       ops.stem8_supported(self.cin, self.cout, self.k, self.stride, self.pad, t, h, w))
        if self.t8:
            xin = Act(self.ctx.storage((key, "t8"), *ops.stem8_plane_dims(n, t, h, w)))
            ops.stem8_input_fold(x_f32, xin.planes)
            return xin
        xin = Act(self.ctx.storage(key, n, t, h, w // 2, 8))
        ops.stem_input_fold(x_f32, xin.planes)
        return xin

    def fprop(self, x: Planes) -> torch.Tensor:
        ctx, g = self.ctx, self.g
        c = self.cout
        self.splits = self.bn.num_splits if (self.sub and ctx.training) else 1
        want_stats = ctx.training and self.splits == 1
        if self.t8:
            n, t, h, w = x.n, x.t // 2, x.h * 2, (x.w // 8 - 1) * 16
            ot, oh, ow = g.out_dims(t, h, w)
            f = ctx.buf((self.name, "z.hi"), (self.k[0] * ops.STEM8_ZG * 64,), torch.bfloat16)
            flo = ctx.buf((self.name, "z.lo"), f.shape, torch.bfloat16) if ctx.nsplit == 3 else None
            ops.stem8_filter_fold(self.conv.weight, f, flo)
            y = ctx.buf((self.name, "y"), (n, ot, oh, ow, c))
            m_tiles = ops.stem8_m_tiles(x, g)
            stats = ctx.buf((self.name, "stats8"), (2, c, m_tiles)) if want_stats else None
            ops.stem8_fprop(x, f, flo, g, y, stats, nsplit=ctx.nsplit)
        else:
            n = x.n
            ot, oh, ow = g.out_dims(x.t, x.h, 2 * x.w)
            f = ctx.buf((self.name, "f.hi"), (self.cout, g.kfold), torch.bfloat16)
            flo = ctx.buf((self.name, "f.lo"), f.shape, torch.bfloat16) if ctx.nsplit == 3 else None
            fm = ops.FilterMat(f, flo, self.cout, g.kfold // 8, 8)
            ops.stem_filter_fold(self.conv.weight, g, fm)
            y = ctx.buf((self.name, "y"), (n, ot, oh, ow, c))
            m_tiles = ops.stem_m_tiles(x, g)
            stats = ctx.buf((self.name, "stats"), (2, c, m_tiles)) if want_stats else None
            ops.stem_fprop(x, fm, g, y, stats, nsplit=ctx.nsplit)
        self.rows_per_clip = ot * oh * ow
        self._bn_forward(y, stats, m_tiles, c, zero=False)
        self.x, self.y = x, y
        return y

    def wgrad(self, dy: Planes) -> None:
        ctx, g = self.ctx, self.g
        dwm = ctx.scratch("dwm", self.cout * g.kfold, F32).view(self.cout, g.kfold)
        ops.zero_f32(ops.f32view(dwm))
        if self.t8:
            ops.stem8_wgrad(self.x, dy, g, dwm, nsplit=ctx.nsplit)
        else:
            ops.stem_wgrad(self.x, dy, g, dwm, nsplit=ctx.nsplit)
        ops.stem_filter_unfold_grad(dwm, ctx.grad_of(self.conv.weight), g)

    def dgrad(self, dy, x_act):
        raise RuntimeError("stem convolutions have no data gradient")


class GraphedProgram:

    def __init__(self, model, inputs: List[torch.Tensor], with_backward: bool = False):
        self.model = model
        self.params = list(model.parameters())
        self.pool = torch.cuda.graph_pool_handle()
        self.static_in = [torch.empty_like(x) for x in inputs]
        for s, x in zip(self.static_in, inputs):
            s.copy_(x)
        self.fwd_graph = torch.cuda.CUDAGraph()
        n0 = ops.launches()
# ... 129 lines not shown
```

slowfast_b200/lib.py:

```python
from __future__ import annotations

import ctypes as C
from pathlib import Path

from .build import lib_path


class NativeLibraryError(RuntimeError):
    pass


class ConvDesc(C.Structure):

    _fields_ = [
        ("a_hi", C.c_void_p), ("a_lo", C.c_void_p),
        ("n", C.c_int32), ("d", C.c_int32), ("h", C.c_int32), ("w", C.c_int32), ("c", C.c_int32),
        ("c_pitch", C.c_int64),
        ("b_hi", C.c_void_p), ("b_lo", C.c_void_p),
        ("cout", C.c_int32),
        ("kt", C.c_int32), ("kh", C.c_int32), ("kw", C.c_int32),
        ("dil_t", C.c_int32), ("dil_h", C.c_int32), ("dil_w", C.c_int32),
        ("str_t", C.c_int32), ("str_h", C.c_int32), ("str_w", C.c_int32),
        ("low_t", C.c_int32), ("low_h", C.c_int32), ("low_w", C.c_int32),
        ("out_t", C.c_int32), ("out_h", C.c_int32), ("out_w", C.c_int32),
        ("out", C.c_void_p),
        ("os_n", C.c_int64), ("os_t", C.c_int64), ("os_h", C.c_int64), ("os_w", C.c_int64),
        ("accumulate", C.c_int32),
        ("stats", C.c_void_p),
        ("nsplit", C.c_int32),
    ]


class WgradDesc(C.Structure):

    _fields_ = [
        ("x_hi", C.c_void_p), ("x_lo", C.c_void_p),
        ("n", C.c_int32), ("d", C.c_int32), ("h", C.c_int32), ("w", C.c_int32), ("c", C.c_int32),
        ("c_pitch", C.c_int64),
        ("dy_hi", C.c_void_p), ("dy_lo", C.c_void_p),
        ("cout", C.c_int32), ("dy_pitch", C.c_int64),
        ("kt", C.c_int32), ("kh", C.c_int32), ("kw", C.c_int32),
        ("dil_t", C.c_int32), ("dil_h", C.c_int32), ("dil_w", C.c_int32),
        ("str_t", C.c_int32), ("str_h", C.c_int32), ("str_w", C.c_int32),
        ("low_t", C.c_int32), ("low_h", C.c_int32), ("low_w", C.c_int32),
        ("out_t", C.c_int32), ("out_h", C.c_int32), ("out_w", C.c_int32),
        ("dw", C.c_void_p),
        ("nsplit", C.c_int32),
    ]


class WgradPlan(C.Structure):

    _fields_ = [(name, C.c_int32) for name in ("direct", "transposed", "tile_rows", "bn", "ck", "tiles", "k_blocks",
                                               "slices", "ctas")]


class BnApplyDesc(C.Structure):
    _fields_ = [
        ("y", C.c_void_p), ("y_pitch", C.c_int64), ("scale", C.c_void_p), ("shift", C.c_void_p),
        ("y2", C.c_void_p), ("y2_pitch", C.c_int64), ("scale2", C.c_void_p), ("shift2", C.c_void_p),
        ("res_hi", C.c_void_p), ("res_lo", C.c_void_p), ("res_pitch", C.c_int64),
        ("out_hi", C.c_void_p), ("out_lo", C.c_void_p), ("out_pitch", C.c_int64),
        ("rows", C.c_int64), ("c", C.c_int32), ("relu", C.c_int32),
        ("splits", C.c_int32), ("rows_per_clip", C.c_int64),
    ]


class BnBwdDesc(C.Structure):
    _fields_ = [
        ("dout", C.c_void_p), ("dout_pitch", C.c_int64),
        ("mask_hi", C.c_void_p), ("mask_pitch", C.c_int64),
        ("y", C.c_void_p), ("y_pitch", C.c_int64),
        ("mean", C.c_void_p), ("invstd", C.c_void_p), ("gamma", C.c_void_p),
        ("dgamma", C.c_void_p), ("dbeta", C.c_void_p), ("accumulate_param_grads", C.c_int32),
        ("training", C.c_int32),
        ("dy_hi", C.c_void_p), ("dy_lo", C.c_void_p), ("dy_pitch", C.c_int64),
        ("dres", C.c_void_p), ("dres_pitch", C.c_int64), ("dres_accumulate", C.c_int32),
        ("partials", C.c_void_p), ("coef", C.c_void_p),
        ("rows", C.c_int64), ("c", C.c_int32), ("c_valid", C.c_int32),
        ("mask_scale", C.c_void_p), ("mask_shift", C.c_void_p),
        ("splits", C.c_int32), ("rows_per_clip", C.c_int64),
    ]


class OptChunk(C.Structure):

    _fields_ = [("param", C.c_void_p), ("offset", C.c_int64), ("count", C.c_int32), ("group", C.c_int32)]


class MomentumChunk(C.Structure):

    _fields_ = [("key", C.c_void_p), ("query", C.c_void_p), ("count", C.c_int64)]


class PoolDesc(C.Structure):
    _fields_ = [
        ("y", C.c_void_p), ("scale", C.c_void_p), ("shift", C.c_void_p),
        ("n", C.c_int32), ("t", C.c_int32), ("h", C.c_int32), ("w", C.c_int32), ("c", C.c_int32),
        ("oh", C.c_int32), ("ow", C.c_int32), ("kh", C.c_int32), ("kw", C.c_int32),
        ("sh", C.c_int32), ("sw", C.c_int32), ("ph", C.c_int32), ("pw", C.c_int32),
        ("out_hi", C.c_void_p), ("out_lo", C.c_void_p), ("out_pitch", C.c_int64),
        ("argmax", C.c_void_p),
        ("dout", C.c_void_p), ("dout_pitch", C.c_int64),
        ("dz", C.c_void_p),
        ("splits", C.c_int32),
    ]


class DwPoolDesc(C.Structure):
    _fields_ = [
        ("src", C.c_void_p), ("src_pitch", C.c_int64), ("src_c0", C.c_int32), ("bias", C.c_void_p),
        ("w", C.c_void_p), ("out", C.c_void_p),
        ("b", C.c_int32), ("heads", C.c_int32), ("hd", C.c_int32), ("t", C.c_int32), ("h", C.c_int32),
        ("w_", C.c_int32), ("ot", C.c_int32), ("oh", C.c_int32), ("ow", C.c_int32),
        ("kt", C.c_int32), ("kh", C.c_int32), ("kw", C.c_int32), ("st", C.c_int32), ("sh", C.c_int32),
        ("sw", C.c_int32), ("has_pool", C.c_int32),
        ("dout", C.c_void_p), ("dsrc", C.c_void_p), ("wpartials", C.c_void_p), ("no_cls", C.c_int32),
    ]


class SoftmaxDesc(C.Structure):
    _fields_ = [
        ("s", C.c_void_p), ("s_pitch", C.c_int64), ("rq", C.c_void_p), ("rq_pitch", C.c_int64),
        ("p_hi", C.c_void_p), ("p_lo", C.c_void_p), ("p_pitch", C.c_int64),
        ("bh", C.c_int32), ("nq", C.c_int32), ("nk", C.c_int32),
        ("qt", C.c_int32), ("qh", C.c_int32), ("qw", C.c_int32), ("kt", C.c_int32), ("kh", C.c_int32),
        ("kw", C.c_int32),
        ("dp", C.c_void_p), ("dp_pitch", C.c_int64),
        ("ds_hi", C.c_void_p), ("ds_lo", C.c_void_p), ("ds_pitch", C.c_int64), ("drq", C.c_void_p),
        ("no_cls", C.c_int32), ("spatial_only", C.c_int32),
    ]


class TokPoolDesc(C.Structure):
    _fields_ = [
        ("x", C.c_void_p), ("out", C.c_void_p), ("argmax", C.c_void_p),
        ("b", C.c_int32), ("c", C.c_int32), ("t", C.c_int32), ("h", C.c_int32), ("w", C.c_int32),
        ("ot", C.c_int32), ("oh", C.c_int32), ("ow", C.c_int32),
        ("kt", C.c_int32), ("kh", C.c_int32), ("kw", C.c_int32), ("st", C.c_int32), ("sh", C.c_int32),
        ("sw", C.c_int32),
        ("dout", C.c_void_p), ("dx", C.c_void_p), ("dx_accumulate", C.c_int32), ("no_cls", C.c_int32),
    ]


class Pool3dDesc(C.Structure):
    _fields_ = [
        ("in_hi", C.c_void_p), ("in_lo", C.c_void_p), ("in_pitch", C.c_int64),
        ("out_hi", C.c_void_p), ("out_lo", C.c_void_p), ("out_pitch", C.c_int64),
        ("argmax", C.c_void_p),
        ("n", C.c_int32), ("t", C.c_int32), ("h", C.c_int32), ("w", C.c_int32), ("c", C.c_int32),
        ("ot", C.c_int32), ("oh", C.c_int32), ("ow", C.c_int32),
        ("kt", C.c_int32), ("kh", C.c_int32), ("kw", C.c_int32), ("st", C.c_int32), ("sh", C.c_int32),
        ("sw", C.c_int32), ("pt", C.c_int32), ("ph", C.c_int32), ("pw", C.c_int32),
        ("dout", C.c_void_p), ("dout_pitch", C.c_int64),
        ("din", C.c_void_p), ("din_pitch", C.c_int64), ("din_accumulate", C.c_int32),
    ]


class StemDesc(C.Structure):
    _fields_ = [
        ("x_hi", C.c_void_p), ("x_lo", C.c_void_p),
        ("n", C.c_int32), ("t", C.c_int32), ("h", C.c_int32), ("wf", C.c_int32),
        ("f_hi", C.c_void_p), ("f_lo", C.c_void_p), ("dy_hi", C.c_void_p), ("dy_lo", C.c_void_p),
        ("cout", C.c_int32), ("kt", C.c_int32), ("kh", C.c_int32), ("kwf", C.c_int32),
        ("str_t", C.c_int32), ("str_h", C.c_int32), ("pad_t", C.c_int32), ("pad_h", C.c_int32),
        ("pad_wf", C.c_int32),
        ("out_t", C.c_int32), ("out_h", C.c_int32), ("out_w", C.c_int32),
        ("out", C.c_void_p), ("stats", C.c_void_p), ("dwm", C.c_void_p),
        ("nsplit", C.c_int32),
    ]


class BgemmDesc(C.Structure):
    _fields_ = [
        ("a_hi", C.c_void_p), ("a_lo", C.c_void_p), ("lda", C.c_int64), ("batch_stride_a", C.c_int64),
        ("a_mn_major", C.c_int32),
        ("b_hi", C.c_void_p), ("b_lo", C.c_void_p), ("ldb", C.c_int64), ("batch_stride_b", C.c_int64),
        ("b_mn_major", C.c_int32),
        ("m", C.c_int32), ("n", C.c_int32), ("k", C.c_int32), ("batch", C.c_int32),
        ("out", C.c_void_p), ("ldd", C.c_int64), ("batch_stride_d", C.c_int64),
        ("alpha", C.c_float), ("accumulate", C.c_int32), ("nsplit", C.c_int32),
    ]


_LIB = None

class DwConvDesc(C.Structure):
    _fields_ = [
        ("x_f32", C.c_void_p), ("x_pitch", C.c_int64),
        ("w", C.c_void_p),
        ("y", C.c_void_p), ("y_pitch", C.c_int64), ("stats", C.c_void_p),
        ("n", C.c_int32), ("t", C.c_int32), ("h", C.c_int32), ("w_", C.c_int32), ("c", C.c_int32),
        ("c_valid", C.c_int32), ("ot", C.c_int32), ("oh", C.c_int32), ("ow", C.c_int32),
        ("kt", C.c_int32), ("kh", C.c_int32), ("kw", C.c_int32), ("st", C.c_int32), ("sh", C.c_int32),
        ("sw", C.c_int32), ("pt", C.c_int32), ("ph", C.c_int32), ("pw", C.c_int32),
        ("dy", C.c_void_p), ("dy_pitch", C.c_int64),
        ("dx", C.c_void_p), ("dx_hi", C.c_void_p), ("dx_lo", C.c_void_p), ("dx_pitch", C.c_int64),
        ("dx_accumulate", C.c_int32),
        ("in_scale", C.c_void_p), ("in_shift", C.c_void_p), ("in_relu", C.c_int32),
    ]


class BnActDesc(C.Structure):
    _fields_ = [
        ("y", C.c_void_p), ("y_pitch", C.c_int64),
        ("scale", C.c_void_p), ("shift", C.c_void_p), ("mean", C.c_void_p), ("invstd", C.c_void_p),
        ("gate", C.c_void_p), ("act", C.c_int32),
        ("rows", C.c_int64), ("rows_per_sample", C.c_int64), ("c", C.c_int32),
        ("out_hi", C.c_void_p), ("out_lo", C.c_void_p), ("out_pitch", C.c_int64),
        ("dout", C.c_void_p), ("dout_pitch", C.c_int64),
        ("partials", C.c_void_p), ("davg", C.c_void_p), ("coef", C.c_void_p),
        ("dy", C.c_void_p), ("dy_pitch", C.c_int64),
    ]


class SeDesc(C.Structure):
    _fields_ = [
        ("n", C.c_int32), ("c", C.c_int32), ("c_pad", C.c_int32), ("f", C.c_int32),
        ("rows_per_sample", C.c_int64), ("tiles_per_sample", C.c_int32), ("m_tiles", C.c_int32),
        ("stats", C.c_void_p), ("scale", C.c_void_p), ("shift", C.c_void_p), ("mean", C.c_void_p),
        ("invstd", C.c_void_p),
        ("w1", C.c_void_p), ("b1", C.c_void_p), ("w2", C.c_void_p), ("b2", C.c_void_p),
        ("ymean", C.c_void_p), ("avg", C.c_void_p), ("hid", C.c_void_p), ("gate", C.c_void_p),
        ("partials", C.c_void_p), ("tiles2_per_sample", C.c_int32),
        ("a12", C.c_void_p), ("do2", C.c_void_p), ("dhid", C.c_void_p), ("davg", C.c_void_p),
        ("gamma", C.c_void_p), ("beta", C.c_void_p),
        ("dw1", C.c_void_p), ("db1", C.c_void_p), ("dw2", C.c_void_p), ("db2", C.c_void_p),
        ("dgamma", C.c_void_p), ("dbeta", C.c_void_p), ("coef", C.c_void_p),
        ("training", C.c_int32), ("has_se", C.c_int32),
    ]


_SIGNATURES = [
    ("sfb_last_error", C.c_char_p, []),
    ("sfb_abi_version", C.c_int, []),
    ("sfb_build_arch", C.c_char_p, []),
    ("sfb_conv_m_tiles", C.c_int64, [C.POINTER(ConvDesc)]),
    ("sfb_conv_ksplit", C.c_int32, [C.POINTER(ConvDesc)]),
    ("sfb_conv_igemm", C.c_int, [C.POINTER(ConvDesc), C.c_void_p]),
    ("sfb_conv_wgrad", C.c_int, [C.POINTER(WgradDesc), C.c_void_p]),
    ("sfb_conv_wgrad_plan", C.c_int, [C.POINTER(WgradDesc), C.c_int32, C.POINTER(WgradPlan)]),
    ("sfb_zero_f32_2d", C.c_int, [C.c_void_p, C.c_int64, C.c_int64, C.c_int64, C.c_void_p]),
    ("sfb_add_f32_2d", C.c_int, [C.c_void_p, C.c_void_p, C.c_int64, C.c_int32, C.c_int64, C.c_int64, C.c_void_p]),
    ("sfb_split_planes", C.c_int, [C.c_void_p, C.c_int64, C.c_int32, C.c_int64, C.c_void_p, C.c_void_p, C.c_int64,
                                   C.c_void_p]),
    ("sfb_input_pack", C.c_int, [C.c_void_p, C.c_int32, C.c_int32, C.c_int32, C.c_int32, C.c_int32, C.c_int32,
                                 C.c_void_p, C.c_void_p, C.c_void_p]),
    ("sfb_filter_pack", C.c_int, [C.c_void_p, C.c_int32, C.c_int32, C.c_int32, C.POINTER(C.c_int32), C.c_int32,
                                  C.c_int32, C.c_int32, C.c_void_p, C.c_void_p, C.c_void_p]),
    ("sfb_filter_unpack_grad", C.c_int, [C.c_void_p, C.c_void_p, C.c_int32, C.c_int32, C.c_int32, C.c_int32,
                                         C.c_int32, C.c_void_p]),
    ("sfb_bn_finalize", C.c_int, [C.c_void_p, C.c_int32, C.c_int32, C.c_int64, C.c_void_p, C.c_void_p, C.c_void_p,
                                  C.c_void_p, C.c_float, C.c_float, C.c_int32, C.c_void_p, C.c_void_p, C.c_void_p,
                                  C.c_void_p, C.c_int32, C.c_void_p]),
    ("sfb_bn_split_stats_tiles", C.c_int32, [C.c_int64, C.c_int64, C.c_int32, C.c_int32]),
    ("sfb_bn_split_stats", C.c_int, [C.c_void_p, C.c_int64, C.c_int64, C.c_int32, C.c_int32, C.c_int64, C.c_void_p,
                                     C.c_void_p]),
    ("sfb_bn_apply", C.c_int, [C.POINTER(BnApplyDesc), C.c_void_p]),
    ("sfb_bn_bwd_blocks", C.c_int32, [C.c_int64, C.c_int32, C.c_int32, C.c_int64]),
    ("sfb_bn_bwd", C.c_int, [C.POINTER(BnBwdDesc), C.c_void_p]),
    ("sfb_bn_relu_maxpool_fwd", C.c_int, [C.POINTER(PoolDesc), C.c_void_p]),
    ("sfb_bn_relu_maxpool_bwd", C.c_int, [C.POINTER(PoolDesc), C.c_void_p]),
    ("sfb_maxpool3d_fwd", C.c_int, [C.POINTER(Pool3dDesc), C.c_void_p]),
    ("sfb_maxpool3d_bwd", C.c_int, [C.POINTER(Pool3dDesc), C.c_void_p]),
    ("sfb_stem_input_fold", C.c_int, [C.c_void_p, C.c_int32, C.c_int32, C.c_int32, C.c_int32, C.c_int32, C.c_void_p,
                                      C.c_void_p, C.c_void_p]),
    ("sfb_stem_filter_fold", C.c_int, [C.c_void_p, C.c_void_p, C.c_int32, C.c_int32, C.c_int32, C.c_int32, C.c_int32,
                                       C.c_int32, C.c_int32, C.c_void_p, C.c_void_p, C.c_void_p, C.c_int32,
                                       C.c_void_p]),
    ("sfb_stem_m_tiles", C.c_int64, [C.POINTER(StemDesc)]),
    ("sfb_stem_fprop", C.c_int, [C.POINTER(StemDesc), C.c_void_p]),
    ("sfb_stem_wgrad", C.c_int, [C.POINTER(StemDesc), C.c_void_p]),
    ("sfb_set_wgrad_direct", C.c_int, [C.c_int32]),
    ("sfb_stem8_supported", C.c_int, [C.POINTER(StemDesc)]),
    ("sfb_stem8_m_tiles", C.c_int64, [C.POINTER(StemDesc)]),
    ("sfb_stem8_input_fold", C.c_int, [C.c_void_p, C.c_int32, C.c_int32, C.c_int32, C.c_int32, C.c_int32, C.c_void_p,
                                       C.c_void_p, C.c_void_p]),
    ("sfb_stem8_filter_fold", C.c_int, [C.c_void_p, C.c_int32, C.c_int32, C.c_void_p, C.c_void_p, C.c_void_p]),
    ("sfb_stem8_fprop", C.c_int, [C.POINTER(StemDesc), C.c_void_p]),
    ("sfb_stem8_wgrad", C.c_int, [C.POINTER(StemDesc), C.c_void_p]),
    ("sfb_gemm_batched", C.c_int, [C.POINTER(BgemmDesc), C.c_void_p]),
    ("sfb_layernorm_fwd", C.c_int, [C.c_void_p, C.c_int64, C.c_int64, C.c_int32, C.c_void_p, C.c_void_p, C.c_float, C.c_void_p, C.c_void_p, C.c_void_p, C.c_int64, C.c_void_p, C.c_void_p, C.c_void_p]),
    ("sfb_rowslab_blocks", C.c_int32, [C.c_int64]),
    ("sfb_layernorm_bwd", C.c_int, [C.c_void_p, C.c_int64, C.c_void_p, C.c_int64, C.c_int64, C.c_int32, C.c_void_p, C.c_void_p, C.c_void_p, C.c_void_p, C.c_int64, C.c_int32, C.c_void_p, C.c_void_p, C.c_int32, C.c_void_p, C.c_void_p]),
    ("sfb_colsum", C.c_int, [C.c_void_p, C.c_int64, C.c_int64, C.c_int32, C.c_void_p, C.c_int32, C.c_void_p, C.c_void_p]),
    ("sfb_tokens_assemble", C.c_int, [C.c_void_p] * 6 + [C.c_int32] * 4 + [C.c_void_p, C.c_void_p]),
    ("sfb_tokens_split_grad", C.c_int, [C.c_void_p, C.c_int32, C.c_int32, C.c_int32, C.c_void_p, C.c_void_p, C.c_void_p, C.c_void_p]),
    ("sfb_segment_slabs", C.c_int32, [C.c_int32, C.c_int32]),
    ("sfb_pos_embed_sep_bwd", C.c_int, [C.c_void_p] + [C.c_int32] * 4 + [C.c_void_p] * 5),
    ("sfb_token_mean_fwd", C.c_int, [C.c_void_p] + [C.c_int32] * 3 + [C.c_void_p] * 3),
    ("sfb_token_mean_bwd", C.c_int, [C.c_void_p] + [C.c_int32] * 3 + [C.c_void_p] * 2),
    ("sfb_token_mean_all_fwd", C.c_int, [C.c_void_p] + [C.c_int32] * 3 + [C.c_void_p] * 3),
    ("sfb_token_mean_all_bwd", C.c_int, [C.c_void_p] + [C.c_int32] * 3 + [C.c_void_p] * 2),
    ("sfb_tokens_assemble_joint", C.c_int, [C.c_void_p] * 4 + [C.c_int32] * 3 + [C.c_void_p, C.c_void_p]),
    ("sfb_pos_embed_joint_bwd", C.c_int, [C.c_void_p] + [C.c_int32] * 3 + [C.c_void_p, C.c_void_p]),
    ("sfb_patchify", C.c_int, [C.c_void_p] + [C.c_int32] * 8 + [C.c_void_p] * 3),
    ("sfb_dwpool_fwd", C.c_int, [C.POINTER(DwPoolDesc), C.c_void_p]),
    ("sfb_dwpool_wgrad_blocks", C.c_int32, [C.POINTER(DwPoolDesc)]),
    ("sfb_dwpool_bwd", C.c_int, [C.POINTER(DwPoolDesc), C.c_void_p, C.c_int32, C.c_void_p]),
    ("sfb_softmax_relpos_fwd", C.c_int, [C.POINTER(SoftmaxDesc), C.c_void_p]),
    ("sfb_softmax_relpos_bwd", C.c_int, [C.POINTER(SoftmaxDesc), C.c_void_p]),
    ("sfb_attn_merge", C.c_int, [C.c_void_p, C.c_void_p, C.c_void_p, C.c_int32, C.c_int32, C.c_int32, C.c_int32, C.c_int32, C.c_void_p, C.c_void_p, C.c_void_p]),
    ("sfb_attn_split_grad", C.c_int, [C.c_void_p, C.c_int32, C.c_int32, C.c_int32, C.c_int32, C.c_int32, C.c_void_p, C.c_void_p, C.c_void_p, C.c_void_p]),
    ("sfb_attn_merge_nocls", C.c_int, [C.c_void_p, C.c_void_p, C.c_void_p, C.c_int32, C.c_int32, C.c_int32, C.c_int32, C.c_int32, C.c_void_p, C.c_void_p, C.c_void_p]),
    ("sfb_attn_split_grad_nocls", C.c_int, [C.c_void_p, C.c_int32, C.c_int32, C.c_int32, C.c_int32, C.c_int32, C.c_void_p, C.c_void_p, C.c_void_p, C.c_void_p]),
    ("sfb_residual_add", C.c_int, [C.c_void_p, C.c_void_p, C.c_void_p, C.c_void_p, C.c_void_p, C.c_int64, C.c_int32, C.c_int64, C.c_void_p, C.c_void_p]),
    ("sfb_bias_gelu", C.c_int, [C.c_void_p, C.c_void_p, C.c_int64, C.c_int32, C.c_void_p, C.c_void_p, C.c_void_p]),
    ("sfb_bias_gelu_bwd", C.c_int, [C.c_void_p, C.c_void_p, C.c_void_p, C.c_int64, C.c_int32, C.c_void_p, C.c_void_p, C.c_void_p, C.c_void_p]),
    ("sfb_scale_split", C.c_int, [C.c_void_p, C.c_void_p, C.c_int64, C.c_int32, C.c_int64, C.c_void_p, C.c_void_p, C.c_void_p, C.c_void_p]),
    ("sfb_token_maxpool_fwd", C.c_int, [C.POINTER(TokPoolDesc), C.c_void_p]),
    ("sfb_token_maxpool_bwd", C.c_int, [C.POINTER(TokPoolDesc), C.c_void_p]),
    ("sfb_global_avgpool_fwd", C.c_int, [C.c_void_p, C.c_void_p, C.c_int64, C.c_int32, C.c_int32, C.c_int32,
                                         C.c_void_p, C.c_int64, C.c_void_p]),
    ("sfb_global_avgpool_bwd", C.c_int, [C.c_void_p, C.c_int64, C.c_int32, C.c_int32, C.c_int32, C.c_void_p,
                                         C.c_int64, C.c_void_p]),
    ("sfb_window_avgpool_fwd", C.c_int, [C.c_void_p, C.c_void_p, C.c_int64] + [C.c_int32] * 8 +
     [C.c_void_p, C.c_int64, C.c_void_p]),
    ("sfb_rows_group_mean", C.c_int, [C.c_void_p, C.c_void_p, C.c_int32, C.c_int32, C.c_int32, C.c_void_p]),
    ("sfb_dropout_fwd", C.c_int, [C.c_void_p, C.c_void_p, C.c_int64, C.c_float, C.c_uint64, C.c_void_p, C.c_void_p]),
    ("sfb_dropout_bwd", C.c_int, [C.c_void_p, C.c_void_p, C.c_int64, C.c_float, C.c_void_p]),
    ("sfb_small_linear_fwd", C.c_int, [C.c_void_p, C.c_void_p, C.c_void_p, C.c_void_p, C.c_int32, C.c_int32,
# ... 88 lines not shown
```

slowfast_b200/nets/resnet.py:

```python
from __future__ import annotations

from typing import List, Optional

import torch
import torch.nn as nn

from .. import ops
from ..config import nsplit_of
from ..engine import Act, ConvBN, Ctx, ModelFunction, Namespace, StemConvBN, bump_num_batches_tracked
from ..ops import F32, Planes
from ..subbn import is_sub_bn, norm_factory, num_splits_of

STAGE_DEPTH = {18: (2, 2, 2, 2), 50: (3, 4, 6, 3), 101: (3, 4, 23, 3)}

TEMPORAL_KERNELS = {
    "2d": [[[1]], [[1]], [[1]], [[1]], [[1]]],
    "c2d": [[[1]], [[1]], [[1]], [[1]], [[1]]],
    "slow_c2d": [[[1]], [[1]], [[1]], [[1]], [[1]]],
    "i3d": [[[5]], [[3]], [[3, 1]], [[3, 1]], [[1, 3]]],
    "slow_i3d": [[[5]], [[3]], [[3, 1]], [[3, 1]], [[1, 3]]],
    "slow": [[[1]], [[1]], [[1]], [[3]], [[3]]],
    "slowfast": [[[1], [5]], [[1], [3]], [[1], [3]], [[3], [3]], [[3], [3]]],
}
POOL1 = {"2d": [[1, 1, 1]], "c2d": [[2, 1, 1]], "slow_c2d": [[1, 1, 1]], "i3d": [[2, 1, 1]], "slow_i3d": [[1, 1, 1]],
# ... 11 lines not shown
        self.conv = _conv(cin, cout, k, stride, pad)
        self.bn = norm(num_features=cout, eps=eps, momentum=mmt)
        self.relu = nn.ReLU(True)
        self.pool_layer = nn.MaxPool3d(kernel_size=[1, 3, 3], stride=[1, 2, 2], padding=[0, 1, 1])


class FuseModule(Namespace):

    def __init__(self, dim_in, ratio, kernel, alpha, eps=1e-5, mmt=0.1, norm=nn.BatchNorm3d):
        super().__init__()
        self.conv_f2s = _conv(dim_in, dim_in * ratio, (kernel, 1, 1), (alpha, 1, 1), (kernel // 2, 0, 0))
        self.bn = norm(num_features=dim_in * ratio, eps=eps, momentum=mmt)
        self.relu = nn.ReLU(True)


class BottleneckModule(Namespace):

    def __init__(self, dim_in, dim_out, temp_k, stride, dim_inner, stride_1x1, eps, mmt, norm=nn.BatchNorm3d):
        super().__init__()
        s1, s3 = (stride, 1) if stride_1x1 else (1, stride)
        self.a = _conv(dim_in, dim_inner, (temp_k, 1, 1), (1, s1, s1), (temp_k // 2, 0, 0))
        self.a_bn = norm(num_features=dim_inner, eps=eps, momentum=mmt)
        self.a_relu = nn.ReLU(True)
        self.b = _conv(dim_inner, dim_inner, (1, 3, 3), (1, s3, s3), (0, 1, 1))
        self.b_bn = norm(num_features=dim_inner, eps=eps, momentum=mmt)
        self.b_relu = nn.ReLU(True)
        self.c = _conv(dim_inner, dim_out, (1, 1, 1), (1, 1, 1), (0, 0, 0))
        self.c.final_conv = True
        self.c_bn = norm(num_features=dim_out, eps=eps, momentum=mmt)
        self.c_bn.transform_final_bn = True


class ResBlockModule(Namespace):

    def __init__(self, name, dim_in, dim_out, temp_k, stride, dim_inner, stride_1x1, ctx: Ctx, eps=1e-5, mmt=0.1,
                 norm=nn.BatchNorm3d):
        super().__init__()
        if dim_in != dim_out or stride != 1:
            self.branch1 = _conv(dim_in, dim_out, (1, 1, 1), (1, stride, stride), (0, 0, 0))
            self.branch1_bn = norm(num_features=dim_out, eps=eps, momentum=mmt)
        self.branch2 = BottleneckModule(dim_in, dim_out, temp_k, stride, dim_inner, stride_1x1, eps, mmt, norm)
        self.relu = nn.ReLU(True)
        self._n = name
        self._ctx = ctx
        self._dim_inner, self._dim_out = dim_inner, dim_out
        object.__setattr__(self, "_units", None)

    def units(self):
        if self._units is None:
            b2, n, ctx = self.branch2, self._n, self._ctx
            u = {"a": ConvBN(n + ".a", b2.a, b2.a_bn, ctx), "b": ConvBN(n + ".b", b2.b, b2.b_bn, ctx),
                 "c": ConvBN(n + ".c", b2.c, b2.c_bn, ctx)}
            if hasattr(self, "branch1"):
                u["s"] = ConvBN(n + ".branch1", self.branch1, self.branch1_bn, ctx)
            object.__setattr__(self, "_units", u)
        return self._units

    def out_dims(self, t, h, w):
        u = self.units()
        return u["b"].out_dims(*u["a"].out_dims(t, h, w))

    def bns(self):
        return [u.bn for u in self.units().values()]

    def run_forward(self, x: Act, out: Act) -> None:
        ctx, u, nm = self._ctx, self.units(), self._n
        n, t, h, w = x.dims
        ya = u["a"].fprop(x.planes)
        xa = Act(ctx.storage((nm, "xa"), *ya.shape))
        ops.bn_apply(ops.f32view(ya), u["a"].scale, u["a"].shift, xa.planes, relu=True, **u["a"].split_kw)
        yb = u["b"].fprop(xa.planes)
        xb = Act(ctx.storage((nm, "xb"), *yb.shape))
        ops.bn_apply(ops.f32view(yb), u["b"].scale, u["b"].shift, xb.planes, relu=True, **u["b"].split_kw)
        yc = u["c"].fprop(xb.planes)
        if "s" in u:
            ys = u["s"].fprop(x.planes)
            ops.bn_apply(ops.f32view(yc), u["c"].scale, u["c"].shift, out.planes, relu=True, y2=ops.f32view(ys),
                         scale2=u["s"].scale, shift2=u["s"].shift, **u["c"].split_kw)
        else:
            ops.bn_apply(ops.f32view(yc), u["c"].scale, u["c"].shift, out.planes, relu=True, res=x.planes,
                         **u["c"].split_kw)
        object.__setattr__(self, "_saved", (x, xa, xb, out))

    def run_backward(self) -> None:
        u = self.units()
        x, xa, xb, out = self._saved
        dout = out.grad_view()
        if "s" in u:
            u["s"].bwd(dout, out.planes, x)
            u["c"].bwd(dout, out.planes, xb)
        else:
            acc = x.s.grad_written
            u["c"].bwd(dout, out.planes, xb, dres=x.grad_view(), dres_accumulate=acc)
            x.s.grad_written = True
        u["b"].bwd(xb.grad_view(), xb.planes, xa)
        u["a"].bwd(xa.grad_view(), xa.planes, x)


NONLOCAL_INSTANTIATIONS = ("softmax", "dot_product")


class NonlocalModule(Namespace):

    def __init__(self, name, dim, dim_inner, pool_size, instantiation, group, ctx: Ctx, eps=1e-5, mmt=0.1,
                 norm=nn.BatchNorm3d):
        super().__init__()
        if instantiation not in NONLOCAL_INSTANTIATIONS:
            raise NotImplementedError(f"Unknown norm type {instantiation}")
        self.conv_theta = nn.Conv3d(dim, dim_inner, kernel_size=1, stride=1, padding=0)
        self.conv_phi = nn.Conv3d(dim, dim_inner, kernel_size=1, stride=1, padding=0)
        self.conv_g = nn.Conv3d(dim, dim_inner, kernel_size=1, stride=1, padding=0)
        self.conv_out = nn.Conv3d(dim_inner, dim, kernel_size=1, stride=1, padding=0)
        self.conv_out.zero_init = False
        self.bn = norm(num_features=dim, eps=eps, momentum=mmt)
        self.bn.transform_final_bn = True
        self.use_pool = pool_size is not None and any(s > 1 for s in pool_size)
        self.pool_size = tuple(int(s) for s in pool_size) if pool_size is not None else None
        if self.use_pool:
            self.pool = nn.MaxPool3d(kernel_size=list(pool_size), stride=list(pool_size), padding=[0, 0, 0])
        assert dim % 8 == 0 and dim_inner % 8 == 0, "Non-local widths must be multiples of 8"
        self.instantiation = instantiation
        self.dim, self.dim_inner, self.group = dim, dim_inner, int(group)
        self._n = name
        self._ctx = ctx
        object.__setattr__(self, "_units", None)

    def units(self):
        if self._units is None:
            n, ctx = self._n, self._ctx
            u = {"theta": ConvBN(n + ".theta", self.conv_theta, None, ctx),
                 "phi": ConvBN(n + ".phi", self.conv_phi, None, ctx),
                 "g": ConvBN(n + ".g", self.conv_g, None, ctx),
                 "out": ConvBN(n + ".out", self.conv_out, self.bn, ctx)}
            object.__setattr__(self, "_units", u)
        return self._units

    def run_forward(self, x: Act, out: Act) -> None:
        ctx, u, nm = self._ctx, self.units(), self._n
        n, t, h, w = x.dims
        c, d, grp = x.c, self.dim_inner, self.group
        if t % grp:
            raise ValueError(f"{nm}: NONLOCAL.GROUP {grp} does not divide the {t} frames of the block's input")
        ng, tg = n * grp, t // grp
        nq = tg * h * w
        xg = Planes(x.s.hi, x.s.lo, ng, tg, h, w, c, x.c0)
        th = Act(ctx.storage((nm, "theta"), n, t, h, w, d))
        ops.bias_split(ops.f32view(u["theta"].fprop(x.planes)), self.conv_theta.bias, th.planes)
        argmax = None
        if self.use_pool:
            k = self.pool_size
            od = (tg // k[0], h // k[1], w // k[2])
            if min(od) < 1:
                raise ValueError(f"{nm}: pool {k} larger than the (grouped) input {(tg, h, w)}")
            src = Act(ctx.storage((nm, "xp"), ng, *od, c))
            argmax = ctx.buf((nm, "argmax"), (ng, *od, c), torch.uint8)
            ops.maxpool3d_fwd(xg, src.planes, argmax, k, k, (0, 0, 0))
        else:
            src = x
        sn, st, sh, sw = src.dims
        nk = sn * st * sh * sw // ng
        ph = Act(ctx.storage((nm, "phi"), sn, st, sh, sw, d))
        gg = Act(ctx.storage((nm, "g"), sn, st, sh, sw, d))
        ops.bias_split(ops.f32view(u["phi"].fprop(src.planes)), self.conv_phi.bias, ph.planes)
        ops.bias_split(ops.f32view(u["g"].fprop(src.planes)), self.conv_g.bias, gg.planes)
        o = ctx.scratch("nl.O", ng * nq * d, F32).view(ng * nq, d)
        nsplit = ctx.nsplit
        if self.instantiation == "softmax":
            nkp = ops.pad8(nk)
            s = ctx.scratch("nl.S", ng * nq * nkp, F32).view(ng * nq, nkp)
            ops.gemm_batched(th.planes, (d, nq * d), False, ph.planes, (d, nk * d), False, nq, nk, d, ng, s, nkp,
                             alpha=d ** -0.5, nsplit=nsplit)
            ps = ctx.storage((nm, "P"), 1, 1, 1, ng * nq, nkp)
            aux = Planes(ps.hi, ps.lo, 1, 1, 1, ng * nq, nkp, 0)
            ops.softmax_relpos_fwd(s, aux, ng, nq, nk)
            ops.gemm_batched(aux, (nkp, nq * nkp), False, gg.planes, (d, nk * d), True, nq, d, nk, ng, o, d, nsplit=nsplit)
        else:
            mf = ctx.scratch("nl.M", ng * d * d, F32).view(ng * d, d)
            ops.gemm_batched(ph.planes, (d, nk * d), True, gg.planes, (d, nk * d), True, d, d, nk, ng, mf, d,
                             nsplit=nsplit)
# ... 25 lines not shown
            nkp = aux.pitch
            dp = ctx.scratch("nl.S", ng * nq * nkp, F32).view(ng * nq, nkp)
            ops.gemm_batched(do, (d, nq * d), False, gg.planes, (d, nk * d), False, nq, nk, d, ng, dp, nkp, nsplit=nsplit)
            ds = ctx.scratch_planes("nl.dS", 1, 1, 1, ng * nq, nkp)
            ops.softmax_relpos_bwd(aux, dp, ds, ng, nq, nk)
            a = d ** -0.5
            ops.gemm_batched(ds, (nkp, nq * nkp), False, ph.planes, (d, nk * d), True, nq, d, nk, ng, dth, d, alpha=a,
                             nsplit=nsplit)
            ops.gemm_batched(ds, (nkp, nq * nkp), True, th.planes, (d, nq * d), True, nk, d, nq, ng, dph, d, alpha=a,
                             nsplit=nsplit)
            ops.gemm_batched(aux, (nkp, nq * nkp), True, do, (d, nq * d), True, nk, d, nq, ng, dg, d, nsplit=nsplit)
        else:
            s = 1.0 / nk
            ops.gemm_batched(do, (d, nq * d), False, aux, (d, d * d), False, nq, d, d, ng, dth, d, alpha=s, nsplit=nsplit)
            dmf = ctx.scratch("nl.M", ng * d * d, F32).view(ng * d, d)
            ops.gemm_batched(th.planes, (d, nq * d), True, do, (d, nq * d), True, d, d, nq, ng, dmf, d, alpha=s,
                             nsplit=nsplit)
            dm = ctx.scratch_planes("nl.dM", 1, 1, 1, ng * d, d)
            ops.bias_split(ops.f32view(dmf), None, dm)
            ops.gemm_batched(gg.planes, (d, nk * d), False, dm, (d, d * d), False, nk, d, d, ng, dph, d, nsplit=nsplit)
            ops.gemm_batched(ph.planes, (d, nk * d), False, dm, (d, d * d), True, nk, d, d, ng, dg, d, nsplit=nsplit)
        for conv, gm in ((self.conv_theta, dth), (self.conv_phi, dph), (self.conv_g, dg)):
            part = ctx.scratch("colsum.part", ops.colsum_blocks(gm.shape[0]) * d, F32)
            ops.colsum(gm, gm.shape[0], d, ctx.grad_of(conv.bias), part)
        n, t, h, w = x.dims
        dthp = ctx.scratch_planes("nl.dthp", n, t, h, w, d)
        dphp = ctx.scratch_planes("nl.dphip", *src.dims, d)
        dgp = ctx.scratch_planes("nl.dgp", *src.dims, d)
        ops.bias_split(ops.f32view(dth), None, dthp)
        ops.bias_split(ops.f32view(dph), None, dphp)
        ops.bias_split(ops.f32view(dg), None, dgp)
        u["theta"].wgrad(dthp)
        u["theta"].dgrad(dthp, x)
        u["phi"].wgrad(dphp)
        u["g"].wgrad(dgp)
        u["phi"].dgrad(dphp, src)
        u["g"].dgrad(dgp, src)
        if self.use_pool:
            k = self.pool_size
            ops.maxpool3d_bwd(src.grad_view(), argmax, xg, src.dims[1:], x.grad_view(), k, k, (0, 0, 0), accumulate=True)


class StageModule(Namespace):

    def __init__(self, name, dim_in, dim_out, dim_inner, temp_kernel_sizes, stride, num_blocks, num_block_temp_kernel,
                 stride_1x1, ctx: Ctx, nonlocal_inds=None, nonlocal_pool=None, nonlocal_group=None,
                 instantiation="softmax", norm=nn.BatchNorm3d):
        super().__init__()
        self.num_pathways = len(num_blocks)
        self.num_blocks = list(num_blocks)
        nonlocal_inds = nonlocal_inds or [[] for _ in num_blocks]
        for p in range(self.num_pathways):
            tks = (temp_kernel_sizes[p] * num_blocks[p])[:num_block_temp_kernel[p]] + \
                [1] * (num_blocks[p] - num_block_temp_kernel[p])
            for i in range(num_blocks[p]):
                blk = ResBlockModule(f"{name}.pathway{p}_res{i}", dim_in[p] if i == 0 else dim_out[p], dim_out[p],
                                     tks[i], stride[p] if i == 0 else 1, dim_inner[p], stride_1x1, ctx, norm=norm)
                self.add_module(f"pathway{p}_res{i}", blk)
                if i in nonlocal_inds[p]:
                    nln = NonlocalModule(f"{name}.pathway{p}_nonlocal{i}", dim_out[p], dim_out[p] // 2, nonlocal_pool[p],
                                         instantiation, nonlocal_group[p], ctx, norm=norm)
                    self.add_module(f"pathway{p}_nonlocal{i}", nln)

    def blocks(self, p) -> List[ResBlockModule]:
        return [getattr(self, f"pathway{p}_res{i}") for i in range(self.num_blocks[p])]

    def nonlocal_after(self, p, i) -> Optional[NonlocalModule]:
        return getattr(self, f"pathway{p}_nonlocal{i}", None)

    def run_block_forward(self, p, i, x: Act, out: Act, key) -> None:
        blk, nln = self.blocks(p)[i], self.nonlocal_after(p, i)
        if nln is None:
            blk.run_forward(x, out)
            return
        n, t, h, w = out.dims
        mid = Act(blk._ctx.storage(key + ("nl_in",), n, t, h, w, out.c))
        blk.run_forward(x, mid)
        nln.run_forward(mid, out)

    def run_block_backward(self, p, i) -> None:
        nln = self.nonlocal_after(p, i)
        if nln is not None:
            nln.run_backward()
        self.blocks(p)[i].run_backward()


class MLPHeadModule(Namespace):

    def __init__(self, dim_in, dim_out, mlp_dim, num_layers):
        super().__init__()
        layers = [nn.Linear(dim_in, mlp_dim, bias=True)]
        for i in range(1, num_layers):
            layers.append(nn.ReLU(inplace=True))
            layers.append(nn.Linear(mlp_dim, dim_out if i == num_layers - 1 else mlp_dim, bias=True))
        for m in layers:
            if isinstance(m, nn.Linear):
                m.xavier_init = True
        self.projection = nn.Sequential(*layers)


def _check_contrastive_head(contrastive) -> int:
    if contrastive is None:
        return 1
    if list(contrastive.get("PREDICTOR_DEPTHS", [])):
        raise NotImplementedError("CONTRASTIVE.PREDICTOR_DEPTHS (predictor MLP heads) is not on the engine path")
    layers = int(contrastive.get("NUM_MLP_LAYERS", 1))
    if layers > 1:
        for opt in ("BN_MLP", "BN_SYNC_MLP"):
            if contrastive.get(opt, False):
                raise NotImplementedError(f"CONTRASTIVE.{opt} (BatchNorm inside the MLP head) is not on the engine path")
    return layers


class BasicHeadModule(Namespace):

    def __init__(self, dim_in, num_classes, dropout_rate, act_func, pool_size=None, contrastive=None):
        super().__init__()
        mlp_layers = _check_contrastive_head(contrastive)
        self.pool_size = [None] * len(dim_in) if pool_size is None else [None if p is None else tuple(p) for p in pool_size]
        for p in range(len(dim_in)):
            self.add_module(f"pathway{p}_avgpool", nn.Identity())
        if dropout_rate > 0.0:
            self.dropout = nn.Dropout(dropout_rate)
        if mlp_layers == 1:
            self.projection = nn.Linear(sum(dim_in), num_classes, bias=True)
        else:
            self.projection = MLPHeadModule(sum(dim_in), num_classes, int(contrastive.MLP_DIM), mlp_layers)
        if act_func not in ("softmax", "none"):
            raise NotImplementedError(f"head activation {act_func!r} is not on the engine path")
        self.act_func = act_func
        self.dropout_rate = dropout_rate
        self.dim_in = list(dim_in)

    def linears(self) -> List[nn.Linear]:
        if isinstance(self.projection, nn.Linear):
            return [self.projection]
        return [m for m in self.projection.projection if isinstance(m, nn.Linear)]


def init_resnet_weights(model: nn.Module, fc_init_std, zero_init_final_bn, zero_init_final_conv) -> None:
    for m in model.modules():
        if isinstance(m, nn.Conv3d):
            if getattr(m, "final_conv", False) and zero_init_final_conv:
                m.weight.data.zero_()
            else:
                nn.init.kaiming_normal_(m.weight, mode="fan_out", nonlinearity="relu")
                if m.bias is not None:
                    m.bias.data.zero_()
        elif isinstance(m, (nn.BatchNorm3d, nn.BatchNorm2d, nn.BatchNorm1d)):
            zero = getattr(m, "transform_final_bn", False) and zero_init_final_bn
            if m.weight is not None:
                m.weight.data.fill_(0.0 if zero else 1.0)
            if m.bias is not None:
                m.bias.data.zero_()
        if isinstance(m, nn.Linear):
            if getattr(m, "xavier_init", False):
                nn.init.kaiming_uniform_(m.weight, a=1)
            else:
                m.weight.data.normal_(mean=0.0, std=fc_init_std)
            if m.bias is not None:
                m.bias.data.zero_()


class _VideoResNetBase(nn.Module):

    num_pathways = 1
    cuda_graphs = True
# ... 300 lines not shown
```

slowfast_b200/ops.py:

```python
from __future__ import annotations

import ctypes as C
import math
from dataclasses import dataclass
from typing import Optional, Sequence, Tuple

import torch

from . import lib as L

BF16 = torch.bfloat16
F32 = torch.float32

_launches = 0


def launches() -> int:
    return _launches


def _count(n: int = 1) -> None:
    global _launches
    _launches += n

# ... 97 lines not shown
    lib = L.load()
    assert x.dtype == F32 and x.is_contiguous() and x.shape[-1] == out.c
    L.check(lib.sfb_split_planes(x.data_ptr(), out.rows, out.c, x.shape[-1], out.hi_ptr(), out.lo_ptr(), out.pitch,
                                 _stream()), "sfb_split_planes")
    _count()


def input_pack(x: torch.Tensor, out: Planes) -> None:
    lib = L.load()
    n, c, t, h, w = x.shape
    assert x.dtype == F32 and x.is_contiguous() and out.pitch == out.c and out.c0 == 0
    L.check(lib.sfb_input_pack(x.data_ptr(), n, c, t, h, w, out.c, out.hi_ptr(), out.lo_ptr(), _stream()),
            "sfb_input_pack")
    _count()


@dataclass
class FilterMat:

    hi: torch.Tensor
    lo: Optional[torch.Tensor]
    rows: int
    ntaps: int
    cols_pad: int


def filter_pack(w: torch.Tensor, out: FilterMat, tapmap: Optional[Sequence[int]] = None,
                transpose: bool = False) -> None:
    lib = L.load()
    assert w.dtype == F32 and w.is_contiguous()
    cout, cin = w.shape[0], w.shape[1]
    taps_total = w[0, 0].numel() if w.dim() > 2 else 1
    ntaps = out.ntaps
    tm = None
    if tapmap is not None:
        assert len(tapmap) == ntaps
        tm = (C.c_int32 * ntaps)(*tapmap)
    L.check(lib.sfb_filter_pack(w.data_ptr(), cout, cin, taps_total, tm, ntaps, 1 if transpose else 0, out.cols_pad,
                                out.hi.data_ptr(), _ptr(out.lo), _stream()), "sfb_filter_pack")
    _count()


def alloc_filter(rows: int, ntaps: int, cols: int, nsplit: int, device) -> FilterMat:
    cp = pad8(cols)
    hi = torch.empty((rows, ntaps * cp), dtype=BF16, device=device)
    lo = torch.empty((rows, ntaps * cp), dtype=BF16, device=device) if nsplit == 3 else None
    return FilterMat(hi, lo, rows, ntaps, cp)


def filter_unpack_grad(dwm: torch.Tensor, dw: torch.Tensor, cin_pad: int, accumulate: bool) -> None:
    lib = L.load()
    cout, cin = dw.shape[0], dw.shape[1]
    taps = dw[0, 0].numel() if dw.dim() > 2 else 1
    assert dw.is_contiguous() and dwm.is_contiguous()
    L.check(lib.sfb_filter_unpack_grad(dwm.data_ptr(), dw.data_ptr(), cout, cin, taps, cin_pad,
                                       1 if accumulate else 0, _stream()), "sfb_filter_unpack_grad")
    _count()


@dataclass
class ConvGeom:

    k: Tuple[int, int, int]
    stride: Tuple[int, int, int] = (1, 1, 1)
    low: Tuple[int, int, int] = (0, 0, 0)
    out: Tuple[int, int, int] = (1, 1, 1)
    dil: Tuple[int, int, int] = (1, 1, 1)


def conv_out_size(i: int, k: int, s: int, p: int, d: int = 1) -> int:
    return (i + 2 * p - d * (k - 1) - 1) // s + 1


def fprop_geom(x: Planes, k, stride, pad, dil=(1, 1, 1)) -> ConvGeom:
    out = tuple(conv_out_size(i, kk, s, p, d) for i, kk, s, p, d in zip((x.t, x.h, x.w), k, stride, pad, dil))
    return ConvGeom(tuple(k), tuple(stride), tuple(-p for p in pad), out, tuple(dil))


def conv_m_tiles(n: int, geom: ConvGeom) -> int:
    m = n * geom.out[0] * geom.out[1] * geom.out[2]
    return (m + 127) // 128


def _conv_desc(x: Planes, f: FilterMat, geom: ConvGeom, out: torch.Tensor, out_strides: Tuple[int, int, int, int],
               out_offset: int, accumulate, stats: Optional[torch.Tensor], nsplit: int):
    assert f.cols_pad == x.c, (f.cols_pad, x.c)
    d = L.ConvDesc()
    d.a_hi, d.a_lo = x.hi_ptr(), x.lo_ptr()
    d.n, d.d, d.h, d.w, d.c, d.c_pitch = x.n, x.t, x.h, x.w, x.c, x.pitch
    d.b_hi, d.b_lo = f.hi.data_ptr(), _ptr(f.lo)
    d.cout = f.rows
    d.kt, d.kh, d.kw = geom.k
    d.dil_t, d.dil_h, d.dil_w = geom.dil
    d.str_t, d.str_h, d.str_w = geom.stride
    d.low_t, d.low_h, d.low_w = geom.low
    d.out_t, d.out_h, d.out_w = geom.out
    d.out = out.data_ptr() + 4 * out_offset
    d.os_n, d.os_t, d.os_h, d.os_w = out_strides
    d.accumulate = int(accumulate)
    d.stats = _ptr(stats)
    d.nsplit = nsplit
    return d


def conv_stats_tiles(x: Planes, f: FilterMat, geom: ConvGeom, out: torch.Tensor,
                     out_strides: Tuple[int, int, int, int], out_offset: int = 0, nsplit: int = 3) -> int:
    d = _conv_desc(x, f, geom, out, out_strides, out_offset, 0, None, nsplit)
    return int(L.load().sfb_conv_m_tiles(C.byref(d)))


def conv_ksplit(x: Planes, f: FilterMat, geom: ConvGeom, out: torch.Tensor, out_strides: Tuple[int, int, int, int],
                out_offset: int = 0, accumulate=0, stats: Optional[torch.Tensor] = None, nsplit: int = 3) -> int:
    d = _conv_desc(x, f, geom, out, out_strides, out_offset, accumulate, stats, nsplit)
    return int(L.load().sfb_conv_ksplit(C.byref(d)))


def conv_igemm(x: Planes, f: FilterMat, geom: ConvGeom, out: torch.Tensor, out_strides: Tuple[int, int, int, int],
               out_offset: int = 0, accumulate: bool = False, stats: Optional[torch.Tensor] = None,
               nsplit: int = 3) -> None:
    lib = L.load()
    d = _conv_desc(x, f, geom, out, out_strides, out_offset, accumulate, stats, nsplit)
    L.check(lib.sfb_conv_igemm(C.byref(d), _stream()), "sfb_conv_igemm")
    _count()


def _wgrad_desc(x: Planes, dy: Planes, geom: ConvGeom, dwm: Optional[torch.Tensor], nsplit: int):
    d = L.WgradDesc()
    d.x_hi, d.x_lo = x.hi_ptr(), x.lo_ptr()
    d.n, d.d, d.h, d.w, d.c, d.c_pitch = x.n, x.t, x.h, x.w, x.c, x.pitch
    d.dy_hi, d.dy_lo = dy.hi_ptr(), dy.lo_ptr()
    d.cout, d.dy_pitch = dy.c, dy.pitch
    d.kt, d.kh, d.kw = geom.k
    d.dil_t, d.dil_h, d.dil_w = geom.dil
    d.str_t, d.str_h, d.str_w = geom.stride
    d.low_t, d.low_h, d.low_w = geom.low
    d.out_t, d.out_h, d.out_w = geom.out
    assert dy.rows == x.n * geom.out[0] * geom.out[1] * geom.out[2]
    d.dw = _ptr(dwm)
    d.nsplit = nsplit
    return d


def conv_wgrad_plan(x: Planes, dy: Planes, geom: ConvGeom, nsplit: int = 3, num_sms: Optional[int] = None):
    if num_sms is None:
        num_sms = torch.cuda.get_device_properties(torch.cuda.current_device()).multi_processor_count
    plan = L.WgradPlan()
    L.check(L.load().sfb_conv_wgrad_plan(C.byref(_wgrad_desc(x, dy, geom, None, nsplit)), num_sms, C.byref(plan)),
            "sfb_conv_wgrad_plan")
    return plan


def conv_wgrad(x: Planes, dy: Planes, geom: ConvGeom, dwm: torch.Tensor, nsplit: int = 3) -> None:
    lib = L.load()
    d = _wgrad_desc(x, dy, geom, dwm, nsplit)
    L.check(lib.sfb_conv_wgrad(C.byref(d), _stream()), "sfb_conv_wgrad")
    _count()


def bn_finalize(partials: Optional[torch.Tensor], m_tiles: int, c: int, count: int, gamma, beta, running_mean,
                running_var, momentum: float, eps: float, training: bool, scale, shift, save_mean, save_invstd,
                affine_c: int = 0):
    lib = L.load()
    L.check(lib.sfb_bn_finalize(_ptr(partials), m_tiles, c, count, _ptr(gamma), _ptr(beta), _ptr(running_mean),
                                _ptr(running_var), momentum, eps, 1 if training else 0, scale.data_ptr(),
                                shift.data_ptr(), _ptr(save_mean), _ptr(save_invstd), affine_c, _stream()),
            "sfb_bn_finalize")
    _count()


def bn_split_stats_tiles(rows: int, rows_per_clip: int, splits: int, c: int) -> int:
    return L.load().sfb_bn_split_stats_tiles(rows, rows_per_clip, splits, c)


def bn_split_stats(y: F32View, splits: int, rows_per_clip: int, partials: torch.Tensor) -> None:
    lib = L.load()
    tiles = bn_split_stats_tiles(y.rows, rows_per_clip, splits, y.c)
    assert partials.dtype == F32 and partials.numel() >= 2 * splits * y.c * tiles
    L.check(lib.sfb_bn_split_stats(y.ptr(), y.pitch, y.rows, y.c, splits, rows_per_clip, partials.data_ptr(),
                                   _stream()), "sfb_bn_split_stats")
    _count()


def bn_apply(y: F32View, scale, shift, out: Planes, relu: bool, y2: Optional[F32View] = None, scale2=None,
             shift2=None, res: Optional[Planes] = None, splits: int = 1, rows_per_clip: int = 0) -> None:
    lib = L.load()
    d = L.BnApplyDesc()
    d.splits, d.rows_per_clip = splits, rows_per_clip
    d.y, d.y_pitch, d.scale, d.shift = y.ptr(), y.pitch, scale.data_ptr(), shift.data_ptr()
    if y2 is not None:
        d.y2, d.y2_pitch, d.scale2, d.shift2 = y2.ptr(), y2.pitch, scale2.data_ptr(), shift2.data_ptr()
    if res is not None:
        assert res.c == out.c and res.rows == out.rows
        d.res_hi, d.res_lo, d.res_pitch = res.hi_ptr(), res.lo_ptr(), res.pitch
    d.out_hi, d.out_lo, d.out_pitch = out.hi_ptr(), out.lo_ptr(), out.pitch
    d.rows, d.c, d.relu = out.rows, out.c, 1 if relu else 0
    assert y.rows == out.rows and y.c == out.c
    L.check(lib.sfb_bn_apply(C.byref(d), _stream()), "sfb_bn_apply")
    _count()


def bn_bwd_blocks(rows: int, c: int, splits: int = 1, rows_per_clip: int = 0) -> int:
    return L.load().sfb_bn_bwd_blocks(rows, c, splits, rows_per_clip)


def bn_bwd_scratch(rows: int, c: int, device, splits: int = 1, rows_per_clip: int = 0):
    nb = bn_bwd_blocks(rows, c, splits, rows_per_clip)
    return (torch.empty((nb, 2, c), dtype=F32, device=device), torch.empty((3, splits * c), dtype=F32, device=device))


def bn_bwd(dout: F32View, mask: Optional[Planes], y: F32View, mean, invstd, gamma, dgamma, dbeta, dy: Planes,
           partials, coef, training: bool = True, accumulate_param_grads: bool = False,
           dres: Optional[F32View] = None, dres_accumulate: bool = False, c_valid: int = 0,
           mask_affine=None, splits: int = 1, rows_per_clip: int = 0) -> None:
    lib = L.load()
    d = L.BnBwdDesc()
    d.c_valid = c_valid
    d.splits, d.rows_per_clip = splits, rows_per_clip
    if mask_affine is not None:
        assert mask is None
        d.mask_scale, d.mask_shift = mask_affine[0].data_ptr(), mask_affine[1].data_ptr()
    d.dout, d.dout_pitch = dout.ptr(), dout.pitch
    if mask is not None:
        d.mask_hi, d.mask_pitch = mask.hi_ptr(), mask.pitch
    d.y, d.y_pitch = y.ptr(), y.pitch
    d.mean, d.invstd, d.gamma = mean.data_ptr(), invstd.data_ptr(), _ptr(gamma)
    d.dgamma, d.dbeta = _ptr(dgamma), _ptr(dbeta)
    d.accumulate_param_grads = 1 if accumulate_param_grads else 0
    d.training = 1 if training else 0
    d.dy_hi, d.dy_lo, d.dy_pitch = dy.hi_ptr(), dy.lo_ptr(), dy.pitch
    if dres is not None:
        d.dres, d.dres_pitch, d.dres_accumulate = dres.ptr(), dres.pitch, 1 if dres_accumulate else 0
    d.partials, d.coef = partials.data_ptr(), coef.data_ptr()
    d.rows, d.c = dy.rows, dy.c
    assert dout.rows == dy.rows and y.rows == dy.rows
    L.check(lib.sfb_bn_bwd(C.byref(d), _stream()), "sfb_bn_bwd")
    _count(3)


def _pool_desc(n, t, h, w, c, oh, ow, k, s, p):
    d = L.PoolDesc()
    d.n, d.t, d.h, d.w, d.c, d.oh, d.ow = n, t, h, w, c, oh, ow
    d.kh, d.kw = k
    d.sh, d.sw = s
    d.ph, d.pw = p
    return d


def bn_relu_maxpool_fwd(y: torch.Tensor, scale, shift, out: Planes, argmax: torch.Tensor, k, s, p,
                        splits: int = 1) -> None:
    lib = L.load()
    n, t, h, w, c = y.shape
    d = _pool_desc(n, t, h, w, c, out.h, out.w, k, s, p)
    d.splits = splits
    d.y, d.scale, d.shift = y.data_ptr(), scale.data_ptr(), shift.data_ptr()
    d.out_hi, d.out_lo, d.out_pitch = out.hi_ptr(), out.lo_ptr(), out.pitch
    d.argmax = argmax.data_ptr()
    L.check(lib.sfb_bn_relu_maxpool_fwd(C.byref(d), _stream()), "sfb_bn_relu_maxpool_fwd")
    _count()


def bn_relu_maxpool_bwd(dout: F32View, argmax: torch.Tensor, dz: torch.Tensor, oh, ow, k, s, p) -> None:
    lib = L.load()
    n, t, h, w, c = dz.shape
    d = _pool_desc(n, t, h, w, c, oh, ow, k, s, p)
    d.argmax = argmax.data_ptr()
    d.dout, d.dout_pitch = dout.ptr(), dout.pitch
    d.dz = dz.data_ptr()
    L.check(lib.sfb_bn_relu_maxpool_bwd(C.byref(d), _stream()), "sfb_bn_relu_maxpool_bwd")
    _count()


def global_avgpool_fwd(x: Planes, out: torch.Tensor, col0: int = 0) -> None:
    lib = L.load()
    assert out.dtype == F32 and out.dim() == 2 and out.is_contiguous()
    L.check(lib.sfb_global_avgpool_fwd(x.hi_ptr(), x.lo_ptr(), x.pitch, x.n, x.t * x.h * x.w, x.c,
                                       out.data_ptr() + 4 * col0, out.shape[1], _stream()), "sfb_global_avgpool_fwd")
    _count()


def global_avgpool_bwd(dpooled: torch.Tensor, col0: int, n: int, spatial: int, c: int, dx: F32View) -> None:
    lib = L.load()
    L.check(lib.sfb_global_avgpool_bwd(dpooled.data_ptr() + 4 * col0, dpooled.shape[1], n, spatial, c, dx.ptr(),
                                       dx.pitch, _stream()), "sfb_global_avgpool_bwd")
    _count()


def window_avgpool_fwd(x: Planes, k: Tuple[int, int, int], out: torch.Tensor, col0: int = 0) -> None:
    lib = L.load()
    assert out.dtype == F32 and out.dim() == 2 and out.is_contiguous()
    L.check(lib.sfb_window_avgpool_fwd(x.hi_ptr(), x.lo_ptr(), x.pitch, x.n, x.t, x.h, x.w, x.c, k[0], k[1], k[2],
                                       out.data_ptr() + 4 * col0, out.shape[1], _stream()), "sfb_window_avgpool_fwd")
    _count()


def rows_group_mean(x: torch.Tensor, out: torch.Tensor, g: int) -> None:
    lib = L.load()
    n, k = out.shape
    assert x.shape == (n * g, k) and x.is_contiguous() and out.is_contiguous()
    L.check(lib.sfb_rows_group_mean(x.data_ptr(), out.data_ptr(), n, g, k, _stream()), "sfb_rows_group_mean")
    _count()


def dropout_fwd(x: torch.Tensor, mask: torch.Tensor, p: float, seed: int,
                step: Optional[torch.Tensor] = None) -> None:
    lib = L.load()
    L.check(lib.sfb_dropout_fwd(x.data_ptr(), mask.data_ptr(), x.numel(), p, seed & (2 ** 64 - 1), _ptr(step),
                                _stream()), "sfb_dropout_fwd")
    _count(2 if step is not None else 1)


def dropout_bwd(dx: torch.Tensor, mask: torch.Tensor, p: float) -> None:
    lib = L.load()
    L.check(lib.sfb_dropout_bwd(dx.data_ptr(), mask.data_ptr(), dx.numel(), p, _stream()), "sfb_dropout_bwd")
    _count()


def small_linear_fwd(x, w, b, y, relu: bool = False) -> None:
    lib = L.load()
    m, j = x.shape
# ... 810 lines not shown
```

Before: 181.3.

## Fuse BN-backward gradient statistics into the dgrad conv epilogue

```diff
diff --git a/include/slowfast_b200.h b/include/slowfast_b200.h
--- a/include/slowfast_b200.h
+++ b/include/slowfast_b200.h
@@ -29,9 +29,20 @@
   int32_t accumulate;
   float* stats;
   int32_t nsplit;
+  int32_t bst_consumers;
+  const float* bst_y[2];
+  const float* bst_mean[2];
+  const float* bst_invstd[2];
+  const float* bst_mask_scale;
+  const float* bst_mask_shift;
+  const void* bst_mask_hi;
+  float* bst_partials;
+  int32_t bst_cols, bst_col0;
 } sfb_conv_desc;
 
 int64_t sfb_conv_m_tiles(const sfb_conv_desc* d);
+int64_t sfb_conv_bst_tiles(const sfb_conv_desc* d);
+int32_t sfb_conv_bst_post(const sfb_conv_desc* d);
 int32_t sfb_conv_ksplit(const sfb_conv_desc* d);
 int sfb_conv_igemm(const sfb_conv_desc* d, void* stream);
 
@@ -118,6 +129,7 @@
   int32_t c_valid;
   const float* mask_scale; const float* mask_shift;
   int32_t splits; int64_t rows_per_clip;
+  int32_t tile_cols; int32_t tile_s2;
 } sfb_bn_bwd_desc;
 int32_t sfb_bn_bwd_blocks(int64_t rows, int32_t c, int32_t splits, int64_t rows_per_clip);
 int sfb_bn_bwd(const sfb_bn_bwd_desc* d, void* stream);
diff --git a/slowfast_b200/csrc/conv_direct.cu b/slowfast_b200/csrc/conv_direct.cu
--- a/slowfast_b200/csrc/conv_direct.cu
+++ b/slowfast_b200/csrc/conv_direct.cu
@@ -155,14 +155,24 @@
   }
 }
 
+static size_t direct_smem(const sfb_conv_desc* d, int coutp) {
+  return (size_t(d->kt * d->kh * d->kw) * d->c * coutp + size_t(8) * coutp + size_t(128) * (coutp + 1)) * sizeof(float) +
+         128 * sizeof(long long) + 8;
+}
+
+bool conv_direct_selects(const sfb_conv_desc* d) {
+  const int64_t macs = int64_t(d->kt) * d->kh * d->kw * d->c * d->cout;
+  int coutp = 8;
+  while (coutp < d->cout) coutp <<= 1;
+  return !(d->c > 8 || d->cout > 64 || macs > 1024 || direct_smem(d, coutp) > 96 * 1024);
+}
+
 int conv_direct_try(const sfb_conv_desc* d, cudaStream_t stream, int* rc_out) {
   const int taps = d->kt * d->kh * d->kw;
-  const int64_t macs = int64_t(taps) * d->c * d->cout;
   int coutp = 8;
   while (coutp < d->cout) coutp <<= 1;
-  const size_t smem = (size_t(taps) * d->c * coutp + size_t(8) * coutp + size_t(128) * (coutp + 1)) * sizeof(float) +
-                      128 * sizeof(long long) + 8;
-  if (d->c > 8 || d->cout > 64 || macs > 1024 || smem > 96 * 1024) return 0;
+  const size_t smem = direct_smem(d, coutp);
+  if (!conv_direct_selects(d)) return 0;
   DirectParams p;
   p.a_hi = (const __nv_bfloat16*)d->a_hi; p.a_lo = (const __nv_bfloat16*)d->a_lo; p.c_pitch = d->c_pitch;
   p.b_hi = (const __nv_bfloat16*)d->b_hi; p.b_lo = (const __nv_bfloat16*)d->b_lo;
diff --git a/slowfast_b200/csrc/conv_igemm.cu b/slowfast_b200/csrc/conv_igemm.cu
--- a/slowfast_b200/csrc/conv_igemm.cu
+++ b/slowfast_b200/csrc/conv_igemm.cu
@@ -1,6 +1,7 @@
 #include <algorithm>
 #include <cstdint>
 #include <cstdio>
+#include <cuda_bf16.h>
 
 #include "../../include/slowfast_b200.h"
 #include "ptx.cuh"
@@ -43,15 +44,44 @@
   int accumulate;
   int epi_coalesced;
   float* stats;
+  const float* bst_y[2];
+  const float* bst_mean[2];
+  const float* bst_invstd[2];
+  const float* bst_mscale;
+  const float* bst_mshift;
+  const __nv_bfloat16* bst_mask;
+  float* bst_part;
+  int bst_cols, bst_col0;
 };
+
+__device__ __forceinline__ bool relu_plane_positive(float y, float scale, float shift) {
+  return __bfloat162float(__float2bfloat16_rn(fmaf(y, scale, shift))) > 0.f;
+}
+__device__ __forceinline__ bool bf16_bits_positive(uint32_t bits16) { return __uint_as_float(bits16 << 16) > 0.f; }
 
 __device__ __forceinline__ int k_block_begin(const ConvParams& p, int kpart) {
   return kpart * p.k_blocks / p.ksplit;
 }
 
 int conv_direct_try(const sfb_conv_desc* d, cudaStream_t stream, int* rc_out);
-
-template <int NSPLIT, int BN>
+bool conv_direct_selects(const sfb_conv_desc* d);
+int64_t bn_bwd_tile_stats_cols(int64_t rows, int c);
+int bn_bwd_tile_stats(const sfb_conv_desc* d, int64_t rows, cudaStream_t stream);
+
+__device__ __forceinline__ void epi_store(float* out, long long off, float4 y, int accumulate) {
+  float4* dst = reinterpret_cast<float4*>(out + off);
+  if (accumulate == 2) {
+    asm volatile("red.global.add.v4.f32 [%0], {%1, %2, %3, %4};" ::"l"(dst), "f"(y.x), "f"(y.y), "f"(y.z), "f"(y.w)
+                 : "memory");
+  } else if (accumulate) {
+    const float4 o = *dst;
+    *dst = make_float4(y.x + o.x, y.y + o.y, y.z + o.z, y.w + o.w);
+  } else {
+    *dst = y;
+  }
+}
+
+template <int NSPLIT, int BN, int BST>
 __global__ void __launch_bounds__(CONV_THREADS, 1) conv_igemm_kernel(const __grid_constant__ ConvParams p) {
   static_assert(BN % 16 == 0 && BN <= BN_MAX, "tile width: a multiple of 16 up to BN_MAX");
   extern __shared__ uint8_t smem_raw[];
@@ -200,6 +230,7 @@
     const int q = ew & 3;
     const int half = ew >> 2;
     long long* roff_s = reinterpret_cast<long long*>(reinterpret_cast<float*>(smem + p.off_staging) + ew * EPI_STAGE_FLOATS);
+    constexpr int RV = BST ? 1 + BST : 2;
     float* red = reinterpret_cast<float*>(smem + p.off_red);
     const int sub = lane >> 2, cq = lane & 3;
     constexpr int nchunks = BN >> 4;
@@ -224,13 +255,120 @@
         roff = on_ * p.os_n + oz_ * p.os_z + op_ * p.os_p + oq_ * p.os_q;
       }
       const uint32_t rmask = __ballot_sync(0xffffffffu, rvalid);
-      float* red_w = red + ((size_t(acc) * 4 + q) * BN) * 2;
+      float* red_w = red + ((size_t(acc) * 4 + q) * BN) * RV;
       roff_s[lane] = roff;
       __syncwarp();
       long long ro[4];
 #pragma unroll
       for (int k = 0; k < 4; ++k) ro[k] = roff_s[k * 8 + sub];
 
+      if constexpr (BST) {
+        if (half >= nchunks) mbar_wait(tfull, it & 1);
+        for (int ch = half; ch < nchunks; ch += 2) {
+          const int c0 = ch * 16;
+          const int limit = min(BN, p.Ntot - ncol0) - c0;
+          const bool cvalid = cq * 4 < limit;
+          const long long cof = ncol0 + c0 + cq * 4;
+          float4 y0v[4];
+          uint2 mv[4];
+#pragma unroll
+          for (int k = 0; k < 4; ++k) {
+            const bool ok = ((rmask >> (k * 8 + sub)) & 1u) && cvalid;
+            y0v[k] = ok ? __ldg(reinterpret_cast<const float4*>(p.bst_y[0] + ro[k] + cof)) : make_float4(0.f, 0.f, 0.f, 0.f);
+            mv[k] = (ok && p.bst_mask) ? __ldg(reinterpret_cast<const uint2*>(p.bst_mask + ro[k] + cof)) : make_uint2(0u, 0u);
+          }
+          float mu[BST][4], is[BST][4], msc[4], msh[4];
+#pragma unroll
+          for (int j = 0; j < BST; ++j) {
+            const float4 m = cvalid ? __ldg(reinterpret_cast<const float4*>(p.bst_mean[j] + cof)) : make_float4(0.f, 0.f, 0.f, 0.f);
+            const float4 v = cvalid ? __ldg(reinterpret_cast<const float4*>(p.bst_invstd[j] + cof)) : make_float4(0.f, 0.f, 0.f, 0.f);
+            mu[j][0] = m.x; mu[j][1] = m.y; mu[j][2] = m.z; mu[j][3] = m.w;
+            is[j][0] = v.x; is[j][1] = v.y; is[j][2] = v.z; is[j][3] = v.w;
+          }
+          if constexpr (BST == 1) {
+            const bool ok = cvalid && p.bst_mscale;
+            const float4 a = ok ? __ldg(reinterpret_cast<const float4*>(p.bst_mscale + cof)) : make_float4(0.f, 0.f, 0.f, 0.f);
+            const float4 b = ok ? __ldg(reinterpret_cast<const float4*>(p.bst_mshift + cof)) : make_float4(0.f, 0.f, 0.f, 0.f);
+            msc[0] = a.x; msc[1] = a.y; msc[2] = a.z; msc[3] = a.w;
+            msh[0] = b.x; msh[1] = b.y; msh[2] = b.z; msh[3] = b.w;
+          }
+          if (ch == half) mbar_wait(tfull, it & 1);
+          float s1[4] = {0.f, 0.f, 0.f, 0.f}, s2[BST][4];
+#pragma unroll
+          for (int j = 0; j < BST; ++j)
+#pragma unroll
+            for (int i = 0; i < 4; ++i) s2[j][i] = 0.f;
+#pragma unroll
+          for (int k = 0; k < 4; ++k) {
+            const int r = k * 8 + sub;
+            const float4 a = *reinterpret_cast<const float4*>(qtile + size_t(r) * p.acc_pitch + c0 + cq * 4);
+            if (((rmask >> r) & 1u) && cvalid) {
+              float4 v = a;
+              float4* dst = reinterpret_cast<float4*>(p.out + ro[k] + cof);
+              if (p.accumulate) {
+                const float4 o = *dst;
+                v = make_float4(a.x + o.x, a.y + o.y, a.z + o.z, a.w + o.w);
+              }
+              *dst = v;
+              float4 y1v = make_float4(0.f, 0.f, 0.f, 0.f);
+              if constexpr (BST == 2) y1v = __ldg(reinterpret_cast<const float4*>(p.bst_y[1] + ro[k] + cof));
+              const float vv[4] = {v.x, v.y, v.z, v.w};
+              const float y0[4] = {y0v[k].x, y0v[k].y, y0v[k].z, y0v[k].w};
+              const float y1[4] = {y1v.x, y1v.y, y1v.z, y1v.w};
+              const uint32_t mb[4] = {mv[k].x & 0xffffu, mv[k].x >> 16, mv[k].y & 0xffffu, mv[k].y >> 16};
+#pragma unroll
+              for (int i = 0; i < 4; ++i) {
+                bool pos = bf16_bits_positive(mb[i]);
+                if constexpr (BST == 1) {
+                  if (p.bst_mscale) pos = relu_plane_positive(y0[i], msc[i], msh[i]);
+                }
+                const float dz = pos ? vv[i] : 0.f;
+                s1[i] += dz;
+                s2[0][i] = fmaf(dz, (y0[i] - mu[0][i]) * is[0][i], s2[0][i]);
+                if constexpr (BST == 2) s2[1][i] = fmaf(dz, (y1[i] - mu[1][i]) * is[1][i], s2[1][i]);
+              }
+            }
+          }
+#pragma unroll
+          for (int i = 0; i < 4; ++i) {
+#pragma unroll
+            for (int o = 4; o <= 16; o <<= 1) {
+              s1[i] += __shfl_xor_sync(0xffffffffu, s1[i], o);
+#pragma unroll
+              for (int j = 0; j < BST; ++j) s2[j][i] += __shfl_xor_sync(0xffffffffu, s2[j][i], o);
+            }
+          }
+          if (sub == 0) {
+#pragma unroll
+            for (int i = 0; i < 4; ++i) {
+              const int cl = c0 + cq * 4 + i;
+              red_w[cl * RV] = s1[i];
+#pragma unroll
+              for (int j = 0; j < BST; ++j) red_w[cl * RV + 1 + j] = s2[j][i];
+            }
+          }
+        }
+        __syncwarp();
+        if (lane == 0) mbar_arrive(tempty);
+        named_bar_sync(1, 32 * EPI_WARPS);
+        const float* rb = red + size_t(acc) * 4 * BN * RV;
+        for (int cl = ew * 32 + lane; cl < BN; cl += 32 * EPI_WARPS) {
+          const int col = ncol0 + cl;
+          if (col < p.Ntot) {
+            float t[RV];
+#pragma unroll
+            for (int j = 0; j < RV; ++j) t[j] = 0.f;
+#pragma unroll
+            for (int w = 0; w < 4; ++w)
+#pragma unroll
+              for (int j = 0; j < RV; ++j) t[j] += rb[(size_t(w) * BN + cl) * RV + j];
+            const size_t c = size_t(p.bst_col0) + mt;
+#pragma unroll
+            for (int j = 0; j < RV; ++j) p.bst_part[(size_t(j) * p.Ntot + col) * p.bst_cols + c] = t[j];
+          }
+        }
+        continue;
+      }
       mbar_wait(tfull, it & 1);
       for (int ch = half; ch < nchunks; ch += 2) {
         const int c0 = ch * 16;
@@ -244,18 +382,7 @@
           s4[0] += y.x; s4[1] += y.y; s4[2] += y.z; s4[3] += y.w;
           q4[0] = fmaf(y.x, y.x, q4[0]); q4[1] = fmaf(y.y, y.y, q4[1]);
           q4[2] = fmaf(y.z, y.z, q4[2]); q4[3] = fmaf(y.w, y.w, q4[3]);
-          if (((rmask >> r) & 1u) && cvalid) {
-            float4* dst = reinterpret_cast<float4*>(p.out + ro[k] + ncol0 + c0 + cq * 4);
-            if (p.accumulate == 2) {
-              asm volatile("red.global.add.v4.f32 [%0], {%1, %2, %3, %4};" ::"l"(dst), "f"(y.x), "f"(y.y), "f"(y.z), "f"(y.w)
-                           : "memory");
-            } else if (p.accumulate) {
-              const float4 o = *dst;
-              *dst = make_float4(y.x + o.x, y.y + o.y, y.z + o.z, y.w + o.w);
-            } else {
-              *dst = y;
-            }
-          }
+          if (((rmask >> r) & 1u) && cvalid) epi_store(p.out, ro[k] + ncol0 + c0 + cq * 4, y, p.accumulate);
         }
         if (p.stats != nullptr) {
 #pragma unroll
@@ -344,12 +471,13 @@
          d->os_n == int64_t(d->out_t) * d->os_t;
 }
 
-static int conv_ksplit(const sfb_conv_desc* d, const ConvGrid& g, bool with_stats) {
+static int conv_ksplit(const sfb_conv_desc* d, const ConvGrid& g, bool with_stats, bool with_bst) {
   const int tiles = g.m_tiles * g.n_tiles;
   const int P = g_num_sms;
   if (P <= 0 || d->c <= 8 || 2 * tiles < P) return 1;
-  if ((d->accumulate == 0 || with_stats) && !rows_regular(d)) return 1;
+  if ((d->accumulate == 0 || with_stats || with_bst) && !rows_regular(d)) return 1;
   if (with_stats && (d->accumulate != 0 || d->cout % 8 != 0 || d->os_w % 4 != 0)) return 1;
+  if (with_bst && d->os_w % 4 != 0) return 1;
   auto cost = [&](int s) { return double((int64_t(tiles) * s + P - 1) / P) / s * (1.0 + 0.02 * (s - 1)); };
   int best = 1;
   for (int s = 2; s <= 8 && 4 * s <= g.k_blocks; ++s)
@@ -363,14 +491,23 @@
 
 extern "C" int64_t sfb_conv_m_tiles(const sfb_conv_desc* d) {
   const ConvGrid g = conv_grid(d);
-  if (device_props() == 0 && conv_ksplit(d, g, true) > 1)
+  if (device_props() == 0 && conv_ksplit(d, g, true, false) > 1)
     return sfb_bn_split_stats_tiles(g.M, g.M, 1, d->cout);
   return g.m_tiles;
 }
 
+extern "C" int32_t sfb_conv_bst_post(const sfb_conv_desc* d) {
+  return conv_direct_selects(d) || (device_props() == 0 && conv_ksplit(d, conv_grid(d), false, true) > 1) ? 1 : 0;
+}
+
+extern "C" int64_t sfb_conv_bst_tiles(const sfb_conv_desc* d) {
+  const ConvGrid g = conv_grid(d);
+  return sfb_conv_bst_post(d) ? bn_bwd_tile_stats_cols(g.M, d->cout) : g.m_tiles;
+}
+
 extern "C" int32_t sfb_conv_ksplit(const sfb_conv_desc* d) {
   if (device_props()) return 1;
-  return conv_ksplit(d, conv_grid(d), d->stats != nullptr);
+  return conv_ksplit(d, conv_grid(d), d->stats != nullptr, d->bst_consumers > 0);
 }
 
 extern "C" int sfb_conv_igemm(const sfb_conv_desc* d, void* stream_) {
@@ -395,9 +532,24 @@
     return -10;
   }
 
+  const bool bst = d->bst_consumers > 0;
+  if (bst) {
+    bool ok = d->bst_consumers <= 2 && (d->bst_consumers == 1 || !d->bst_mask_scale) && d->accumulate != 2 && d->stats == nullptr && d->cout % 8 == 0 &&
+              d->bst_partials && (d->bst_mask_scale ? d->bst_mask_shift != nullptr : d->bst_mask_hi != nullptr) &&
+              d->bst_col0 >= 0 && d->bst_col0 + sfb_conv_bst_tiles(d) <= d->bst_cols;
+    for (int k = 0; k < d->bst_consumers; ++k) ok = ok && d->bst_y[k] && d->bst_mean[k] && d->bst_invstd[k];
+    if (!ok) {
+      set_error("sfb_conv_igemm: backward statistics need 1-2 consumers with y / mean / invstd, a mask (two consumers: "
+                "a plane), accumulate 0 or "
+                "1, cout a multiple of 8 and columns [%d, %d + %lld) within %d", d->bst_col0, d->bst_col0,
+                (long long)sfb_conv_bst_tiles(d), d->bst_cols);
+      return -10;
+    }
+  }
   {
     int rc_direct = 0;
-    if (conv_direct_try(d, stream, &rc_direct)) return rc_direct;
+    if (conv_direct_try(d, stream, &rc_direct))
+      return rc_direct == 0 && bst ? bn_bwd_tile_stats(d, M64, stream) : rc_direct;
   }
   ConvParams p;
   memset(&p, 0, sizeof(p));
@@ -429,7 +581,7 @@
   p.BN = g.BN;
   p.n_tiles = g.n_tiles;
   p.m_tiles = g.m_tiles;
-  p.ksplit = conv_ksplit(d, g, d->stats != nullptr);
+  p.ksplit = conv_ksplit(d, g, d->stats != nullptr, bst);
   p.chunk_bytes = BLOCK_M * p.CK * 2;
   p.b_bytes = p.BN * 128;
   p.a_plane_bytes = (uint32_t(p.cps) * p.chunk_bytes + 1023u) / 1024u * 1024u;
@@ -450,7 +602,8 @@
   }
   p.acc_pitch = uint32_t(p.BN) + 4;
   const uint32_t acc_bytes = BLOCK_M * p.acc_pitch * 4;
-  const uint32_t tail = acc_bytes + EPI_WARPS * EPI_STAGE_FLOATS * 4 + 2 * 4 * p.BN * 2 * 4 + 256;
+  const uint32_t red_bytes = 2 * 4 * p.BN * (bst ? 1 + d->bst_consumers : 2) * 4;
+  const uint32_t tail = acc_bytes + EPI_WARPS * EPI_STAGE_FLOATS * 4 + red_bytes + 256;
   const uint32_t budget = uint32_t(g_smem_optin) - 1024 - tail;
   p.stages = std::min<int>(MAX_STAGES, budget / p.stage_bytes);
   p.stages = std::min(p.stages, std::max(2, p.k_blocks * 4));
@@ -462,7 +615,7 @@
   p.off_acc = p.stages * p.stage_bytes;
   p.off_staging = p.off_acc + acc_bytes;
   p.off_red = p.off_staging + EPI_WARPS * EPI_STAGE_FLOATS * 4;
-  p.off_bars = p.off_red + 2 * 4 * p.BN * 2 * 4;
+  p.off_bars = p.off_red + red_bytes;
   const uint32_t smem_bytes = p.off_bars + 256 + 1024;
   p.out = d->out;
   p.os_n = d->os_n;
@@ -472,6 +625,20 @@
   p.accumulate = p.ksplit > 1 ? 2 : d->accumulate;
   p.epi_coalesced = 1;
   p.stats = p.ksplit > 1 ? nullptr : d->stats;
+  const bool bst_epi = bst && p.ksplit == 1;
+  if (bst_epi) {
+    for (int k = 0; k < d->bst_consumers; ++k) {
+      p.bst_y[k] = d->bst_y[k];
+      p.bst_mean[k] = d->bst_mean[k];
+      p.bst_invstd[k] = d->bst_invstd[k];
+    }
+    p.bst_mscale = d->bst_mask_scale;
+    p.bst_mshift = d->bst_mask_shift;
+    p.bst_mask = d->bst_mask_scale ? nullptr : static_cast<const __nv_bfloat16*>(d->bst_mask_hi);
+    p.bst_part = d->bst_partials;
+    p.bst_cols = d->bst_cols;
+    p.bst_col0 = d->bst_col0;
+  }
 
   const int lower[3] = {d->low_w, d->low_h, d->low_t};
   const int strd[3] = {d->str_w, d->str_h, d->str_t};
@@ -513,18 +680,20 @@
   const int grid = std::min(units, g_num_sms * ctas_per_sm);
   {
     typedef void (*KernelFn)(const ConvParams);
-#define SFB_CONV_FNS(S) {conv_igemm_kernel<S, 16>, conv_igemm_kernel<S, 32>, conv_igemm_kernel<S, 48>, \
-                         conv_igemm_kernel<S, 64>, conv_igemm_kernel<S, 80>, conv_igemm_kernel<S, 96>, \
-                         conv_igemm_kernel<S, 112>, conv_igemm_kernel<S, 128>}
-    static const KernelFn fns[2][BN_MAX / 16] = {SFB_CONV_FNS(1), SFB_CONV_FNS(3)};
+#define SFB_CONV_FNS(S, T) {conv_igemm_kernel<S, 16, T>, conv_igemm_kernel<S, 32, T>, conv_igemm_kernel<S, 48, T>, \
+                            conv_igemm_kernel<S, 64, T>, conv_igemm_kernel<S, 80, T>, conv_igemm_kernel<S, 96, T>, \
+                            conv_igemm_kernel<S, 112, T>, conv_igemm_kernel<S, 128, T>}
+    static const KernelFn fns[3][2][BN_MAX / 16] = {{SFB_CONV_FNS(1, 0), SFB_CONV_FNS(3, 0)},
+                                                    {SFB_CONV_FNS(1, 1), SFB_CONV_FNS(3, 1)},
+                                                    {SFB_CONV_FNS(1, 2), SFB_CONV_FNS(3, 2)}};
 #undef SFB_CONV_FNS
-    static bool attr[2][BN_MAX / 16] = {};
-    const int a = d->nsplit == 3 ? 1 : 0, b = p.BN / 16 - 1;
-    if (!attr[a][b]) {
-      cudaFuncSetAttribute(fns[a][b], cudaFuncAttributeMaxDynamicSharedMemorySize, g_smem_optin);
-      attr[a][b] = true;
-    }
-    fns[a][b]<<<grid, CONV_THREADS, smem_bytes, stream>>>(p);
+    static bool attr[3][2][BN_MAX / 16] = {};
+    const int e = bst_epi ? d->bst_consumers : 0, a = d->nsplit == 3 ? 1 : 0, b = p.BN / 16 - 1;
+    if (!attr[e][a][b]) {
+      cudaFuncSetAttribute(fns[e][a][b], cudaFuncAttributeMaxDynamicSharedMemorySize, g_smem_optin);
+      attr[e][a][b] = true;
+    }
+    fns[e][a][b]<<<grid, CONV_THREADS, smem_bytes, stream>>>(p);
   }
   cudaError_t e = cudaGetLastError();
   if (e != cudaSuccess) {
@@ -534,5 +703,6 @@
   }
   if (p.ksplit > 1 && d->stats != nullptr)
     return sfb_bn_split_stats(d->out, d->os_w, p.M, d->cout, 1, p.M, d->stats, stream);
+  if (bst && !bst_epi) return bn_bwd_tile_stats(d, p.M, stream);
   return 0;
 }
diff --git a/slowfast_b200/csrc/elementwise.cu b/slowfast_b200/csrc/elementwise.cu
--- a/slowfast_b200/csrc/elementwise.cu
+++ b/slowfast_b200/csrc/elementwise.cu
@@ -481,6 +481,165 @@
   if (dbeta) dbeta[ch] = accumulate ? dbeta[ch] + float(t1) : float(t1);
 }
 
+__global__ void __launch_bounds__(256) bn_bwd_finalize_tiles_kernel(const float* __restrict__ partials, int cols, int c,
+                                                                    int s2, double count, const float* __restrict__ gamma,
+                                                                    const float* __restrict__ invstd,
+                                                                    float* __restrict__ dgamma, float* __restrict__ dbeta,
+                                                                    int accumulate, int training,
+                                                                    float* __restrict__ coef, int c_valid) {
+  __shared__ double sm1[256], sm2[256];
+  const int ch = blockIdx.x;
+  if (ch >= c_valid) {
+    if (threadIdx.x == 0) coef[ch] = coef[c + ch] = coef[2 * c + ch] = 0.f;
+    return;
+  }
+  const float* p1 = partials + size_t(ch) * cols;
+  const float* p2 = partials + (size_t(s2) * c + ch) * cols;
+  double t1 = 0.0, t2 = 0.0;
+#pragma unroll 4
+  for (int i = threadIdx.x; i < cols; i += 256) {
+    t1 += double(p1[i]);
+    t2 += double(p2[i]);
+  }
+  sm1[threadIdx.x] = t1;
+  sm2[threadIdx.x] = t2;
+  __syncthreads();
+  for (int o = 128; o > 0; o >>= 1) {
+    if (threadIdx.x < o) {
+      sm1[threadIdx.x] += sm1[threadIdx.x + o];
+      sm2[threadIdx.x] += sm2[threadIdx.x + o];
+    }
+    __syncthreads();
+  }
+  if (threadIdx.x != 0) return;
+  const double S1 = sm1[0], S2 = sm2[0];
+  const double a = double(gamma ? gamma[ch] : 1.f) * double(invstd[ch]);
+  coef[ch] = float(a);
+  coef[c + ch] = training ? float(a * S1 / count) : 0.f;
+  coef[2 * c + ch] = training ? float(a * S2 / count) : 0.f;
+  if (dgamma) dgamma[ch] = accumulate ? dgamma[ch] + float(S2) : float(S2);
+  if (dbeta) dbeta[ch] = accumulate ? dbeta[ch] + float(S1) : float(S1);
+}
+
+__host__ __device__ inline int64_t bn_bwd_tile_rows(int c) { return split_stats_chunk(c); }
+struct BwdTileStatsParams {
+  const float* dout; int64_t os_n, os_t, os_h, os_w;
+  int ot, oh, ow;
+  int64_t rows; int64_t chunk_rows;
+  int c, consumers;
+  const float* y[2]; const float* mean[2]; const float* invstd[2];
+  const float* mask_scale; const float* mask_shift; const __nv_bfloat16* mask;
+  float* partials; int cols, col0;
+};
+__device__ __forceinline__ bool relu_plane_positive(float y, float scale, float shift) {
+  return __bfloat162float(__float2bfloat16_rn(fmaf(y, scale, shift))) > 0.f;
+}
+__global__ void __launch_bounds__(256) bn_bwd_tile_stats_kernel(const BwdTileStatsParams p) {
+  extern __shared__ float sm[];
+  const int cg = p.c / 8;
+  const int lanes_c = cg < int(blockDim.x) ? cg : int(blockDim.x);
+  const int lanes_r = blockDim.x / lanes_c;
+  const int lc = threadIdx.x % lanes_c;
+  const int lr = threadIdx.x / lanes_c;
+  const int64_t r0 = int64_t(blockIdx.x) * p.chunk_rows;
+  const int64_t r1 = min(r0 + p.chunk_rows, p.rows);
+  for (int g0 = 0; g0 < cg; g0 += lanes_c) {
+    const int g = g0 + lc;
+    float s1[8], s2[2][8];
+#pragma unroll
+    for (int k = 0; k < 8; ++k) s1[k] = s2[0][k] = s2[1][k] = 0.f;
+    if (g < cg && lr < lanes_r) {
+      const int c = g * 8;
+      float mu[2][8], is[2][8], msc[8], msh[8];
+      for (int j = 0; j < p.consumers; ++j) {
+        load8(p.mean[j] + c, mu[j]);
+        load8(p.invstd[j] + c, is[j]);
+      }
+      if (p.mask_scale) {
+        load8(p.mask_scale + c, msc);
+        load8(p.mask_shift + c, msh);
+      }
+      for (int64_t r = r0 + lr; r < r1; r += lanes_r) {
+        int64_t t = r;
+        const int q = int(t % p.ow); t /= p.ow;
+        const int h = int(t % p.oh); t /= p.oh;
+        const int z = int(t % p.ot);
+        const int64_t off = (t / p.ot) * p.os_n + z * p.os_t + h * p.os_h + q * p.os_w + c;
+        float d[8], y0[8];
+        load8(p.dout + off, d);
+        load8(p.y[0] + off, y0);
+        if (p.mask_scale) {
+#pragma unroll
+          for (int k = 0; k < 8; ++k) d[k] = relu_plane_positive(y0[k], msc[k], msh[k]) ? d[k] : 0.f;
+        } else {
+          float m[8];
+          load_planes8(p.mask + off, nullptr, m);
+#pragma unroll
+          for (int k = 0; k < 8; ++k) d[k] = m[k] > 0.f ? d[k] : 0.f;
+        }
+#pragma unroll
+        for (int k = 0; k < 8; ++k) {
+          s1[k] += d[k];
+          s2[0][k] = fmaf(d[k], (y0[k] - mu[0][k]) * is[0][k], s2[0][k]);
+        }
+        if (p.consumers > 1) {
+          float y1[8];
+          load8(p.y[1] + off, y1);
+#pragma unroll
+          for (int k = 0; k < 8; ++k) s2[1][k] = fmaf(d[k], (y1[k] - mu[1][k]) * is[1][k], s2[1][k]);
+        }
+      }
+    }
+#pragma unroll
+    for (int k = 0; k < 8; ++k) {
+      sm[threadIdx.x * 24 + k] = s1[k];
+      sm[threadIdx.x * 24 + 8 + k] = s2[0][k];
+      sm[threadIdx.x * 24 + 16 + k] = s2[1][k];
+    }
+    __syncthreads();
+    if (lr == 0 && g < cg) {
+      for (int q = 1; q < lanes_r; ++q) {
+#pragma unroll
+        for (int k = 0; k < 8; ++k) {
+          s1[k] += sm[(q * lanes_c + lc) * 24 + k];
+          s2[0][k] += sm[(q * lanes_c + lc) * 24 + 8 + k];
+          s2[1][k] += sm[(q * lanes_c + lc) * 24 + 16 + k];
+        }
+      }
+      const int64_t col = p.col0 + blockIdx.x;
+#pragma unroll
+      for (int k = 0; k < 8; ++k) {
+        const int64_t ch = g * 8 + k;
+        p.partials[ch * p.cols + col] = s1[k];
+        for (int j = 0; j < p.consumers; ++j) p.partials[((1 + j) * int64_t(p.c) + ch) * p.cols + col] = s2[j][k];
+      }
+    }
+    __syncthreads();
+  }
+}
+
+int64_t bn_bwd_tile_stats_cols(int64_t rows, int c) { return (rows + bn_bwd_tile_rows(c) - 1) / bn_bwd_tile_rows(c); }
+
+int bn_bwd_tile_stats(const sfb_conv_desc* d, int64_t rows, cudaStream_t stream) {
+  BwdTileStatsParams p;
+  p.dout = d->out; p.os_n = d->os_n; p.os_t = d->os_t; p.os_h = d->os_h; p.os_w = d->os_w;
+  p.ot = d->out_t; p.oh = d->out_h; p.ow = d->out_w;
+  p.rows = rows; p.chunk_rows = bn_bwd_tile_rows(d->cout);
+  p.c = d->cout; p.consumers = d->bst_consumers;
+  for (int j = 0; j < 2; ++j) {
+    p.y[j] = j < d->bst_consumers ? d->bst_y[j] : nullptr;
+    p.mean[j] = j < d->bst_consumers ? d->bst_mean[j] : nullptr;
+    p.invstd[j] = j < d->bst_consumers ? d->bst_invstd[j] : nullptr;
+  }
+  p.mask_scale = d->bst_mask_scale; p.mask_shift = d->bst_mask_shift;
+  p.mask = (const __nv_bfloat16*)d->bst_mask_hi;
+  p.partials = d->bst_partials; p.cols = d->bst_cols; p.col0 = d->bst_col0;
+  const int64_t blocks = bn_bwd_tile_stats_cols(rows, d->cout);
+  bn_bwd_tile_stats_kernel<<<unsigned(blocks), 256, 256 * 24 * sizeof(float), stream>>>(p);
+  SFB_LAUNCH_CHECK("sfb_conv_igemm(backward statistics)");
+  return 0;
+}
+
 struct BnBwdApplyParams {
   const float* dout; int64_t dout_pitch;
   const __nv_bfloat16* mask; int64_t mask_pitch;
@@ -829,22 +988,34 @@
   }
   if (!split_geometry_ok("sfb_bn_bwd", d->rows, d->splits, d->rows_per_clip)) return -10;
   const int splits = d->splits > 1 ? d->splits : 1;
-  const int nblocks = sfb_bn_bwd_blocks(d->rows, d->c, splits, d->rows_per_clip);
-  const int bpc = splits > 1 ? bn_bwd_blocks_per_clip(d->rows, d->rows_per_clip) : 1;
-  BnBwdReduceParams r;
-  r.dout = d->dout; r.dout_pitch = d->dout_pitch;
-  r.mask = (const bf16*)d->mask_hi; r.mask_pitch = d->mask_pitch;
-  r.mask_scale = d->mask_scale; r.mask_shift = d->mask_shift;
-  r.y = d->y; r.y_pitch = d->y_pitch; r.mean = d->mean; r.invstd = d->invstd;
-  r.rows = d->rows; r.c = d->c; r.partials = d->partials;
-  r.splits = splits; r.rows_per_clip = d->rows_per_clip; r.blocks_per_clip = bpc;
-  bn_bwd_reduce_kernel<<<nblocks, 256, 256 * 16 * sizeof(float), stream>>>(r);
-  SFB_LAUNCH_CHECK("sfb_bn_bwd(reduce)");
-  bn_bwd_finalize_kernel<<<d->c, 64, 0, stream>>>(d->partials, nblocks, d->c, double(d->rows / splits), d->gamma,
-                                                                 d->invstd, d->dgamma, d->dbeta, d->accumulate_param_grads,
-                                                                 d->training, d->coef,
-                                                                 d->c_valid > 0 ? d->c_valid : d->c, splits, bpc);
-  SFB_LAUNCH_CHECK("sfb_bn_bwd(finalize)");
+  if (d->tile_cols > 0) {
+    if (splits > 1 || d->tile_s2 < 1 || d->tile_s2 > 2) {
+      set_error("sfb_bn_bwd: tile partials need splits 1 and S2 row 1 or 2 (got %d, %d)", splits, d->tile_s2);
+      return -10;
+    }
+    bn_bwd_finalize_tiles_kernel<<<d->c, 256, 0, stream>>>(d->partials, d->tile_cols, d->c, d->tile_s2,
+                                                           double(d->rows), d->gamma, d->invstd, d->dgamma, d->dbeta,
+                                                           d->accumulate_param_grads, d->training, d->coef,
+                                                           d->c_valid > 0 ? d->c_valid : d->c);
+    SFB_LAUNCH_CHECK("sfb_bn_bwd(finalize tiles)");
+  } else {
+    const int nblocks = sfb_bn_bwd_blocks(d->rows, d->c, splits, d->rows_per_clip);
+    const int bpc = splits > 1 ? bn_bwd_blocks_per_clip(d->rows, d->rows_per_clip) : 1;
+    BnBwdReduceParams r;
+    r.dout = d->dout; r.dout_pitch = d->dout_pitch;
+    r.mask = (const bf16*)d->mask_hi; r.mask_pitch = d->mask_pitch;
+    r.mask_scale = d->mask_scale; r.mask_shift = d->mask_shift;
+    r.y = d->y; r.y_pitch = d->y_pitch; r.mean = d->mean; r.invstd = d->invstd;
+    r.rows = d->rows; r.c = d->c; r.partials = d->partials;
+    r.splits = splits; r.rows_per_clip = d->rows_per_clip; r.blocks_per_clip = bpc;
+    bn_bwd_reduce_kernel<<<nblocks, 256, 256 * 16 * sizeof(float), stream>>>(r);
+    SFB_LAUNCH_CHECK("sfb_bn_bwd(reduce)");
+    bn_bwd_finalize_kernel<<<d->c, 64, 0, stream>>>(d->partials, nblocks, d->c, double(d->rows / splits), d->gamma,
+                                                    d->invstd, d->dgamma, d->dbeta, d->accumulate_param_grads,
+                                                    d->training, d->coef, d->c_valid > 0 ? d->c_valid : d->c, splits,
+                                                    bpc);
+    SFB_LAUNCH_CHECK("sfb_bn_bwd(finalize)");
+  }
   BnBwdApplyParams a;
   a.dout = d->dout; a.dout_pitch = d->dout_pitch;
   a.mask = (const bf16*)d->mask_hi; a.mask_pitch = d->mask_pitch;
diff --git a/slowfast_b200/engine.py b/slowfast_b200/engine.py
--- a/slowfast_b200/engine.py
+++ b/slowfast_b200/engine.py
@@ -172,6 +172,9 @@
 
 def _t3(v) -> Tuple[int, int, int]:
     return tuple(int(x) for x in v)
+
+
+BST_MIN_K = 512
 
 
 class ConvBN:
@@ -252,16 +255,23 @@
         return y
 
     def bwd(self, dout: F32View, mask: Optional[Planes], x_act: Optional[Act], dres: Optional[F32View] = None,
-            dres_accumulate: bool = False, mask_from_y: bool = False) -> None:
+            dres_accumulate: bool = False, mask_from_y: bool = False,
+            stats: Optional[Tuple[ops.BnGradStats, int]] = None,
+            consumers: Optional[Tuple[List["ConvBN"], Optional[Planes]]] = None) -> Optional[ops.BnGradStats]:
         ctx = self.ctx
         n, ot, oh, ow, c = self.y.shape
         dy = ctx.scratch_planes("dy", n, ot, oh, ow, c)
-        partials, coef = self._bwd_scratch(n * ot * oh * ow, c)
+        if stats is None:
+            partials, coef = self._bwd_scratch(n * ot * oh * ow, c)
+            tile = None
+        else:
+            coef = self.ctx.scratch("bnb.coef", 3 * c, F32).view(3, c)
+            partials, tile = stats[0].partials, (stats[0].cols, stats[1])
         bn = self.bn
         ops.bn_bwd(dout, mask, ops.f32view(self.y), self.mean, self.invstd, bn.weight, ctx.grad_of(bn.weight),
                    ctx.grad_of(bn.bias), dy, partials, coef, training=ctx.training, dres=dres,
                    dres_accumulate=dres_accumulate, c_valid=self.cout,
-                   mask_affine=(self.scale, self.shift) if mask_from_y else None, **self.split_kw)
+                   mask_affine=(self.scale, self.shift) if mask_from_y else None, tile_stats=tile, **self.split_kw)
         if self.bias is not None:
             rows = n * ot * oh * ow
             dyf = ctx.scratch("bias.dy", rows * c, F32).view(rows, c)
@@ -270,7 +280,8 @@
             ops.colsum(dyf, rows, self.cout, ctx.grad_of(self.bias), part, pitch=c)
         self.wgrad(dy)
         if x_act is not None:
-            self.dgrad(dy, x_act)
+            return self.dgrad(dy, x_act, consumers)
+        return None
 
     def _bwd_scratch(self, rows, c):
         nb = ops.bn_bwd_blocks(rows, c, self.splits, self.rows_per_clip)
@@ -289,7 +300,8 @@
             ops.conv_wgrad(self.x, dy, self.geom, dwm, nsplit=ctx.nsplit)
             ops.filter_unpack_grad(dwm, gw, self.cin_pad, accumulate=False)
 
-    def dgrad(self, dy: Planes, x_act: Act) -> None:
+    def dgrad(self, dy: Planes, x_act: Act,
+              consumers: Optional[Tuple[List["ConvBN"], Optional[Planes]]] = None) -> Optional[ops.BnGradStats]:
         ctx = self.ctx
         _, t, h, w, pitch = x_act.s.shape
         plan = dgrad_plan((t, h, w), self.k, self.stride, self.pad)
@@ -297,18 +309,44 @@
         g = x_act.s.ensure_grad()
         if plan.needs_zero_fill and not acc:
             ops.zero_f32(x_act.grad_view())
+        cp = ops.pad8(self.cout)
+        views = []
         for sub in plan.subs:
             ntap = len(sub.tapmap)
-            cp = ops.pad8(self.cout)
             f = ctx.scratch("dgf.hi", self.cin * ntap * cp, torch.bfloat16).view(self.cin, ntap * cp)
             flo = ctx.scratch("dgf.lo", self.cin * ntap * cp, torch.bfloat16).view(self.cin, ntap * cp) \
                 if ctx.nsplit == 3 else None
-            fm = ops.FilterMat(f, flo, self.cin, ntap, cp)
+            off, strides = dgrad_out_view((t, h, w), self.stride, sub, pitch, x_act.c0)
+            views.append((sub, ops.FilterMat(f, flo, self.cin, ntap, cp),
+                          ops.ConvGeom(sub.k, (1, 1, 1), sub.low, sub.out), off, strides))
+        bst = self._grad_stats(dy, views, x_act, g, acc and plan.needs_zero_fill, consumers)
+        col0 = 0
+        for sub, fm, geom, off, strides in views:
             ops.filter_pack(self.conv.weight, fm, tapmap=sub.tapmap, transpose=True)
-            off, strides = dgrad_out_view((t, h, w), self.stride, sub, pitch, x_act.c0)
-            ops.conv_igemm(dy, fm, ops.ConvGeom(sub.k, (1, 1, 1), sub.low, sub.out), g, strides, out_offset=off,
-                           accumulate=2 if acc else 0, nsplit=ctx.nsplit)
+            if bst is None:
+                ops.conv_igemm(dy, fm, geom, g, strides, out_offset=off, accumulate=2 if acc else 0, nsplit=ctx.nsplit)
+                continue
+            bst.col0 = col0
+            col0 += ops.conv_bst_tiles(dy, fm, geom, g, strides, out_offset=off, nsplit=ctx.nsplit)
+            ops.conv_igemm(dy, fm, geom, g, strides, out_offset=off, accumulate=1 if acc else 0, nsplit=ctx.nsplit,
+                           bst=bst)
         x_act.s.grad_written = True
+        return bst
+
+    def _grad_stats(self, dy: Planes, views, x_act: Act, g: torch.Tensor, partial: bool,
+                    consumers: Optional[Tuple[List["ConvBN"], Optional[Planes]]]) -> Optional[ops.BnGradStats]:
+        if consumers is None or partial or self.taps * self.cout < BST_MIN_K:
+            return None
+        units, mask = consumers
+        if any(u.splits != 1 or u.y is None or u.y.shape != g.shape or u.cout != self.cin for u in units):
+            return None
+        if x_act.c != self.cin or (mask is not None and (mask.hi.shape != g.shape or mask.c0 != x_act.c0)):
+            return None
+        cols = sum(ops.conv_bst_tiles(dy, fm, geom, g, strides, out_offset=off, nsplit=self.ctx.nsplit)
+                   for _, fm, geom, off, strides in views)
+        part = self.ctx.scratch("bst.partials", (1 + len(units)) * self.cin * cols, F32)
+        return ops.BnGradStats(part, cols, [u.y for u in units], [u.mean for u in units], [u.invstd for u in units],
+                               mask=mask, mask_affine=(units[0].scale, units[0].shift) if mask is None else None)
 
 
 class StemConvBN(ConvBN):
diff --git a/slowfast_b200/lib.py b/slowfast_b200/lib.py
--- a/slowfast_b200/lib.py
+++ b/slowfast_b200/lib.py
@@ -28,6 +28,11 @@
         ("accumulate", C.c_int32),
         ("stats", C.c_void_p),
         ("nsplit", C.c_int32),
+        ("bst_consumers", C.c_int32),
+        ("bst_y", C.c_void_p * 2), ("bst_mean", C.c_void_p * 2), ("bst_invstd", C.c_void_p * 2),
+        ("bst_mask_scale", C.c_void_p), ("bst_mask_shift", C.c_void_p), ("bst_mask_hi", C.c_void_p),
+        ("bst_partials", C.c_void_p),
+        ("bst_cols", C.c_int32), ("bst_col0", C.c_int32),
     ]
 
 
@@ -80,6 +85,7 @@
         ("rows", C.c_int64), ("c", C.c_int32), ("c_valid", C.c_int32),
         ("mask_scale", C.c_void_p), ("mask_shift", C.c_void_p),
         ("splits", C.c_int32), ("rows_per_clip", C.c_int64),
+        ("tile_cols", C.c_int32), ("tile_s2", C.c_int32),
     ]
 
 
@@ -237,6 +243,8 @@
     ("sfb_build_arch", C.c_char_p, []),
     ("sfb_conv_m_tiles", C.c_int64, [C.POINTER(ConvDesc)]),
     ("sfb_conv_ksplit", C.c_int32, [C.POINTER(ConvDesc)]),
+    ("sfb_conv_bst_tiles", C.c_int64, [C.POINTER(ConvDesc)]),
+    ("sfb_conv_bst_post", C.c_int32, [C.POINTER(ConvDesc)]),
     ("sfb_conv_igemm", C.c_int, [C.POINTER(ConvDesc), C.c_void_p]),
     ("sfb_conv_wgrad", C.c_int, [C.POINTER(WgradDesc), C.c_void_p]),
     ("sfb_conv_wgrad_plan", C.c_int, [C.POINTER(WgradDesc), C.c_int32, C.POINTER(WgradPlan)]),
diff --git a/slowfast_b200/nets/resnet.py b/slowfast_b200/nets/resnet.py
--- a/slowfast_b200/nets/resnet.py
+++ b/slowfast_b200/nets/resnet.py
@@ -117,19 +117,26 @@
                          **u["c"].split_kw)
         object.__setattr__(self, "_saved", (x, xa, xb, out))
 
-    def run_backward(self) -> None:
+    def out_consumers(self):
+        u = self.units()
+        return [u["c"], u["s"]] if "s" in u else [u["c"]], self._saved[3].planes
+
+    def run_backward(self, stats: Optional[ops.BnGradStats] = None,
+                     prev: Optional["ResBlockModule"] = None) -> Optional[ops.BnGradStats]:
         u = self.units()
         x, xa, xb, out = self._saved
         dout = out.grad_view()
         if "s" in u:
-            u["s"].bwd(dout, out.planes, x)
-            u["c"].bwd(dout, out.planes, xb)
+            u["s"].bwd(dout, out.planes, x, stats=stats and (stats, 2))
+            sb = u["c"].bwd(dout, out.planes, xb, stats=stats and (stats, 1), consumers=([u["b"]], None))
         else:
             acc = x.s.grad_written
-            u["c"].bwd(dout, out.planes, xb, dres=x.grad_view(), dres_accumulate=acc)
+            sb = u["c"].bwd(dout, out.planes, xb, dres=x.grad_view(), dres_accumulate=acc, stats=stats and (stats, 1),
+                            consumers=([u["b"]], None))
             x.s.grad_written = True
-        u["b"].bwd(xb.grad_view(), xb.planes, xa)
-        u["a"].bwd(xa.grad_view(), xa.planes, x)
+        sa = u["b"].bwd(xb.grad_view(), xb.planes, xa, stats=sb and (sb, 1), consumers=([u["a"]], None))
+        return u["a"].bwd(xa.grad_view(), xa.planes, x, stats=sa and (sa, 1),
+                          consumers=prev.out_consumers() if prev is not None else None)
 
 
 NONLOCAL_INSTANTIATIONS = ("softmax", "dot_product")
@@ -321,7 +328,12 @@
         nln = self.nonlocal_after(p, i)
         if nln is not None:
             nln.run_backward()
-        self.blocks(p)[i].run_backward()
+        handed = self.__dict__.pop("_handed_stats", None)
+        stats = handed[1] if handed is not None and handed[0] == (p, i) else None
+        prev = self.blocks(p)[i - 1] if i > 0 and self.nonlocal_after(p, i - 1) is None else None
+        taken = self.blocks(p)[i].run_backward(stats, prev)
+        if taken is not None:
+            object.__setattr__(self, "_handed_stats", ((p, i - 1), taken))
 
 
 class MLPHeadModule(Namespace):
diff --git a/slowfast_b200/ops.py b/slowfast_b200/ops.py
--- a/slowfast_b200/ops.py
+++ b/slowfast_b200/ops.py
@@ -203,8 +203,22 @@
     return (m + 127) // 128
 
 
+@dataclass
+class BnGradStats:
+
+    partials: torch.Tensor
+    cols: int
+    y: Sequence[torch.Tensor]
+    mean: Sequence[torch.Tensor]
+    invstd: Sequence[torch.Tensor]
+    mask: Optional[Planes] = None
+    mask_affine: Optional[Tuple[torch.Tensor, torch.Tensor]] = None
+    col0: int = 0
+
+
 def _conv_desc(x: Planes, f: FilterMat, geom: ConvGeom, out: torch.Tensor, out_strides: Tuple[int, int, int, int],
-               out_offset: int, accumulate, stats: Optional[torch.Tensor], nsplit: int):
+               out_offset: int, accumulate, stats: Optional[torch.Tensor], nsplit: int,
+               bst: Optional[BnGradStats] = None):
     assert f.cols_pad == x.c, (f.cols_pad, x.c)
     d = L.ConvDesc()
     d.a_hi, d.a_lo = x.hi_ptr(), x.lo_ptr()
@@ -221,6 +235,22 @@
     d.accumulate = int(accumulate)
     d.stats = _ptr(stats)
     d.nsplit = nsplit
+    if bst is not None:
+        k = len(bst.y)
+        assert 1 <= k <= 2 and len(bst.mean) == k and len(bst.invstd) == k
+        assert all(y.shape == out.shape and y.dtype == F32 for y in bst.y), "y must share the output's layout"
+        d.bst_consumers = k
+        for j in range(k):
+            d.bst_y[j] = bst.y[j].data_ptr() + 4 * out_offset
+            d.bst_mean[j], d.bst_invstd[j] = bst.mean[j].data_ptr(), bst.invstd[j].data_ptr()
+        if bst.mask_affine is not None:
+            assert bst.mask is None
+            d.bst_mask_scale, d.bst_mask_shift = bst.mask_affine[0].data_ptr(), bst.mask_affine[1].data_ptr()
+        else:
+            assert bst.mask.hi.shape == out.shape, "the mask planes must share the output's layout"
+            d.bst_mask_hi = bst.mask.hi.data_ptr() + 2 * out_offset
+        d.bst_partials, d.bst_cols, d.bst_col0 = bst.partials.data_ptr(), bst.cols, bst.col0
+        assert bst.partials.dtype == F32 and bst.partials.numel() >= (1 + k) * f.rows * bst.cols
     return d
 
 
@@ -236,13 +266,20 @@
     return int(L.load().sfb_conv_ksplit(C.byref(d)))
 
 
+def conv_bst_tiles(x: Planes, f: FilterMat, geom: ConvGeom, out: torch.Tensor,
+                   out_strides: Tuple[int, int, int, int], out_offset: int = 0, nsplit: int = 3) -> int:
+    d = _conv_desc(x, f, geom, out, out_strides, out_offset, 0, None, nsplit)
+    d.bst_consumers = 1
+    return int(L.load().sfb_conv_bst_tiles(C.byref(d)))
+
+
 def conv_igemm(x: Planes, f: FilterMat, geom: ConvGeom, out: torch.Tensor, out_strides: Tuple[int, int, int, int],
                out_offset: int = 0, accumulate: bool = False, stats: Optional[torch.Tensor] = None,
-               nsplit: int = 3) -> None:
-    lib = L.load()
-    d = _conv_desc(x, f, geom, out, out_strides, out_offset, accumulate, stats, nsplit)
+               nsplit: int = 3, *, bst: Optional[BnGradStats] = None) -> None:
+    lib = L.load()
+    d = _conv_desc(x, f, geom, out, out_strides, out_offset, accumulate, stats, nsplit, bst)
     L.check(lib.sfb_conv_igemm(C.byref(d), _stream()), "sfb_conv_igemm")
-    _count()
+    _count(1 + (lib.sfb_conv_bst_post(C.byref(d)) if bst is not None else 0))
 
 
 def _wgrad_desc(x: Planes, dy: Planes, geom: ConvGeom, dwm: Optional[torch.Tensor], nsplit: int):
@@ -332,7 +369,7 @@
 def bn_bwd(dout: F32View, mask: Optional[Planes], y: F32View, mean, invstd, gamma, dgamma, dbeta, dy: Planes,
            partials, coef, training: bool = True, accumulate_param_grads: bool = False,
            dres: Optional[F32View] = None, dres_accumulate: bool = False, c_valid: int = 0,
-           mask_affine=None, splits: int = 1, rows_per_clip: int = 0) -> None:
+           mask_affine=None, splits: int = 1, rows_per_clip: int = 0, tile_stats: Optional[Tuple[int, int]] = None) -> None:
     lib = L.load()
     d = L.BnBwdDesc()
     d.c_valid = c_valid
@@ -353,9 +390,11 @@
         d.dres, d.dres_pitch, d.dres_accumulate = dres.ptr(), dres.pitch, 1 if dres_accumulate else 0
     d.partials, d.coef = partials.data_ptr(), coef.data_ptr()
     d.rows, d.c = dy.rows, dy.c
+    if tile_stats is not None:
+        d.tile_cols, d.tile_s2 = tile_stats
     assert dout.rows == dy.rows and y.rows == dy.rows
     L.check(lib.sfb_bn_bwd(C.byref(d), _stream()), "sfb_bn_bwd")
-    _count(3)
+    _count(2 if tile_stats is not None else 3)
 
 
 def _pool_desc(n, t, h, w, c, oh, ow, k, s, p):
```

Measured after the change: 181.8 (median of 6 runs). Within noise of the previous version (+0.3%).
